# modelscope/dash-infer

Measured on NVIDIA H100. Metric: decode tokens/sec/GPU Qwen2-7B int4-IQ b=1..64; HBM GB/s vs roofline, higher is better.
Workload: dtype bf16 activations x int4 weights (fp32 accumulate), none KV

## Files before the change

### dash-infer_b200/csrc/wq_gemm.cu

```cuda
#include <cstdio>
#include <cstdlib>
#include <cstring>
#include <map>
#include <mutex>
#include <new>

#include "b2_common.cuh"
#include "comm_shared.cuh"
#include "wq_gemm_shared.cuh"

namespace b2 {

constexpr int kWarps = 8;
constexpr int kThreads = kWarps * 32 + 32;
constexpr int kStageBytes = 8192;
static_assert(kBN == kWarps * 16, "one n16 tile per consumer warp");

struct GemmParams {
  const uint8_t* packed;
  const float2* sz;
  const __nv_bfloat16* A;
  int64_t lda;
  __nv_bfloat16* C;
  int64_t ldc;
  const __nv_bfloat16* bias;
  const __nv_bfloat16* residual;
  float* ws;
  unsigned* counters;
  int M, N, K, Np, KT, NG, S;
  int group_tiles;
  int quanta;
  int xt;
  int nst_log2;
  int act;
  float alpha;
  const float* norm_sumsq;
  const __nv_bfloat16* norm_gamma;
  int norm_parts;
  int cluster;
  int norm_self;
  float norm_inv_hidden, norm_eps;
  float* sumsq_out;
  int comm_on;
  CommDev comm;
};

template <int WBITS>
struct WTraits {
  static constexpr int LB = WBITS == 4 ? 16 : (WBITS == 8 ? 32 : 64);
  static constexpr int NCH = LB / 16;
  static constexpr int TILE_BYTES = kWarps * 32 * LB;
  static constexpr int TPS = kStageBytes / TILE_BYTES > 0 ? kStageBytes / TILE_BYTES : 1;
  static constexpr int STAGE_BYTES = TPS * TILE_BYTES;
};

__device__ __forceinline__ void named_bar_sync(int id, int n) { asm volatile("bar.sync %0, %1;" ::"r"(id), "r"(n) : "memory"); }

template <int WBITS, int MT, bool H>
__device__ __forceinline__ void tile_mma(float (&acc)[MT][4], uint32_t wtile, uint32_t woff0, uint32_t woff1, uint32_t xaddr,
                                         int XS8) {
  uint4 xb[MT][2];
#pragma unroll
  for (int m = 0; m < MT; ++m) {
    xb[m][0] = lds128(xaddr + m * XS8);
    xb[m][1] = lds128(xaddr + m * XS8 + 16);
  }
  if (WBITS == 4) {
    const uint2 w0 = lds64(wtile + woff0), w1 = lds64(wtile + woff1);
    const uint32_t r0w[2] = {w0.x, w0.y}, r1w[2] = {w1.x, w1.y};
#pragma unroll
    for (int j = 0; j < 2; ++j) {
      const uint32_t u = r0w[j], v = r1w[j];
      const uint32_t p0 = lop3_and_or(u, kMask4, Ft<H>::kMagic), q0 = lop3_and_or(v, kMask4, Ft<H>::kMagic);
      const uint32_t p1 = lop3_and_or(__funnelshift_r(u, u, 4), kMask4, Ft<H>::kMagic), q1 = lop3_and_or(__funnelshift_r(v, v, 4), kMask4, Ft<H>::kMagic);
      const uint32_t p2 = lop3_and_or(__funnelshift_r(u, u, 8), kMask4, Ft<H>::kMagic), q2 = lop3_and_or(__funnelshift_r(v, v, 8), kMask4, Ft<H>::kMagic);
      const uint32_t p3 = lop3_and_or(__funnelshift_r(u, u, 12), kMask4, Ft<H>::kMagic), q3 = lop3_and_or(__funnelshift_r(v, v, 12), kMask4, Ft<H>::kMagic);
#pragma unroll
      for (int m = 0; m < MT; ++m) {
        Ft<H>::mma(acc[m], p0, q0, p1, q1, xb[m][j].x, xb[m][j].y);
        Ft<H>::mma(acc[m], p2, q2, p3, q3, xb[m][j].z, xb[m][j].w);
      }
    }
  } else if (WBITS == 8) {
    const uint4 w0 = lds128(wtile + woff0), w1 = lds128(wtile + woff1);
    const uint32_t r0w[4] = {w0.x, w0.y, w0.z, w0.w}, r1w[4] = {w1.x, w1.y, w1.z, w1.w};
#pragma unroll
    for (int j = 0; j < 4; ++j) {
      const uint32_t u = r0w[j], v = r1w[j];
      const uint32_t l0 = lop3_and_or(u, kMask4, Ft<H>::kMagic), m0 = lop3_and_or(v, kMask4, Ft<H>::kMagic);
      const uint32_t h0 = lop3_and_or(__funnelshift_r(u, u, 4), kMask4, Ft<H>::kMagicHi), n0 = lop3_and_or(__funnelshift_r(v, v, 4), kMask4, Ft<H>::kMagicHi);
      const uint32_t l1 = lop3_and_or(__funnelshift_r(u, u, 8), kMask4, Ft<H>::kMagic), m1 = lop3_and_or(__funnelshift_r(v, v, 8), kMask4, Ft<H>::kMagic);
      const uint32_t h1 = lop3_and_or(__funnelshift_r(u, u, 12), kMask4, Ft<H>::kMagicHi), n1 = lop3_and_or(__funnelshift_r(v, v, 12), kMask4, Ft<H>::kMagicHi);
#pragma unroll
      for (int m = 0; m < MT; ++m) {
        const uint32_t b0 = (j & 1) ? xb[m][j >> 1].z : xb[m][j >> 1].x;
        const uint32_t b1 = (j & 1) ? xb[m][j >> 1].w : xb[m][j >> 1].y;
        Ft<H>::mma(acc[m], l0, m0, l1, m1, b0, b1);
        Ft<H>::mma(acc[m], h0, n0, h1, n1, b0, b1);
      }
    }
  } else {
#pragma unroll
    for (int u = 0; u < 2; ++u) {
      const uint4 w0 = lds128(wtile + woff0 + u * 2048), w1 = lds128(wtile + woff1 + u * 2048);
#pragma unroll
      for (int m = 0; m < MT; ++m) {
        Ft<H>::mma(acc[m], w0.x, w1.x, w0.y, w1.y, xb[m][u].x, xb[m][u].y);
        Ft<H>::mma(acc[m], w0.z, w1.z, w0.w, w1.w, xb[m][u].z, xb[m][u].w);
      }
    }
  }
}

B2_TRACE_DECL(g_gemv_tr)
#ifdef B2_TRACE
extern "C" int b2_debug_trace_gemv(unsigned long long* host_out) { return (int)cudaMemcpyFromSymbol(host_out, g_gemv_tr, sizeof(g_gemv_tr)); }
#endif

template <int WBITS, int MT, bool GROUPED, bool H>
__global__ void __launch_bounds__(kThreads) wq_gemm_kernel(const GemmParams p) {
  using T = WTraits<WBITS>;
  using F = Ft<H>;
  constexpr int MP = 8 * MT;
  const int NST = 1 << p.nst_log2;
  extern __shared__ __align__(128) uint8_t smem[];
  const int tid = threadIdx.x;
  const int warp = tid >> 5, lane = tid & 31;
  const int g = lane >> 2, t = lane & 3;

  const int ng = blockIdx.x / p.S;
  const int s = blockIdx.x - ng * p.S;
  const int gt = GROUPED ? p.group_tiles : 1;
  const int q0 = (int)((int64_t)s * p.quanta / p.S), q1 = (int)((int64_t)(s + 1) * p.quanta / p.S);
  const int kt0 = q0 * gt, kt1 = q1 * gt;
  const int nt = kt1 - kt0;

  uint8_t* ring = smem;
  const int ring_bytes = NST * T::STAGE_BYTES;
  const int XS = p.xt * 128 + 16;
  uint8_t* xs = ring + ring_bytes;
  uint8_t* grow = xs + MP * XS;
  float* fs = reinterpret_cast<float*>(grow + XS);
  float* suma = fs + MP * kBN;
  const int gpc = GROUPED ? p.xt / gt : 1;
  float* sinv = suma + MP * gpc;
  float* srs = sinv + MP;
  uint64_t* full = reinterpret_cast<uint64_t*>((reinterpret_cast<uintptr_t>(srs + MP + 4) + 7) & ~uintptr_t(7));
  uint64_t* empty = full + NST;
  uint64_t* xbar = empty + NST;
  uint64_t* gbar = xbar + 1;
  __shared__ int s_is_last;

  const bool tr0 = blockIdx.x == 0 && tid == 0;
  if (tr0) B2_TR(g_gemv_tr, 0);
  if (tid == 0) {
    for (int i = 0; i < NST; ++i) {
      mbar_init(&full[i], 1);
      mbar_init(&empty[i], kWarps);
    }
    mbar_init(xbar, 1);
    mbar_init(gbar, 1);
    fence_mbar_init();
  }
  __syncthreads();
  pdl_launch_dependents();
  if (tr0) B2_TR(g_gemv_tr, 1);

  if (warp == kWarps) {
    if (lane == 0) {
      const uint8_t* wsrc = p.packed + ((size_t)ng * p.KT + kt0) * T::TILE_BYTES;
      const int nstages_total = (nt + T::TPS - 1) / T::TPS;
      for (int i = 0; i < nstages_total; ++i) {
        const int slot = i & (NST - 1);
        if (i >= NST) mbar_wait(&empty[slot], ((i >> p.nst_log2) & 1) ^ 1);
        const int tiles = min(T::TPS, nt - i * T::TPS);
        const uint32_t bytes = tiles * T::TILE_BYTES;
        mbar_arrive_expect_tx(&full[slot], bytes);
        bulk_g2s(ring + slot * T::STAGE_BYTES, wsrc + (size_t)i * T::STAGE_BYTES, bytes, &full[slot]);
        if (blockIdx.x == 0 && i == 0) B2_TR(g_gemv_tr, 2);
      }
    }
    return;
  }

  const int n0 = ng * kBN + warp * 16 + g;
  float2 sz0 = make_float2(1.f, 0.f), sz1 = make_float2(1.f, 0.f);
  if (!GROUPED && WBITS != 16) {
    sz0 = p.sz[n0];
    sz1 = p.sz[n0 + 8];
  }

  float acc[MT][4], facc[MT][4];
#pragma unroll
  for (int m = 0; m < MT; ++m)
#pragma unroll
    for (int c = 0; c < 4; ++c) acc[m][c] = facc[m][c] = 0.f;

  for (int i = p.M * XS + tid * 16; i < MP * XS; i += kWarps * 32 * 16) *reinterpret_cast<uint4*>(xs + i) = make_uint4(0, 0, 0, 0);
  const int64_t k_first = (int64_t)kt0 * kBK;
  if (p.norm_self && tid == 0) {
    const int64_t left = ((int64_t)p.K - k_first) * 2;
    const uint32_t gb = (uint32_t)max((int64_t)0, min((int64_t)min(p.xt, nt) * 128, left));
    mbar_arrive_expect_tx(gbar, gb);
    if (gb) bulk_g2s(grow, p.norm_gamma + k_first, gb, gbar);
  }

  pdl_wait();
  if (tr0) B2_TR(g_gemv_tr, 3);

  if (p.norm_sumsq) {
    for (int m = warp; m < MP; m += kWarps) {
      float ss = 0.f;
      if (m < p.M)
        for (int i = lane; i < p.norm_parts; i += 32) ss += __ldcg(p.norm_sumsq + (size_t)i * p.M + m);
#pragma unroll
      for (int o = 16; o > 0; o >>= 1) ss += __shfl_xor_sync(0xffffffffu, ss, o);
      if (lane == 0) sinv[m] = rsqrtf(ss * p.norm_inv_hidden + p.norm_eps);
    }
    named_bar_sync(1, kWarps * 32);
  }
  const uint32_t w_ring = smem_u32(ring);
  const int wc = WBITS == 4 ? (t >> 1) : (WBITS == 8 ? t : 2 * t);
  const int wr = warp * 16 + g;
  const uint32_t woff0 = wc * 2048 + ((wr ^ tile_swz(WBITS, wc)) << 4) + (WBITS == 4 ? 8 * (t & 1) : 0);
  const uint32_t woff1 = wc * 2048 + (((wr + 8) ^ tile_swz(WBITS, wc)) << 4) + (WBITS == 4 ? 8 * (t & 1) : 0);
  const uint32_t x_thr = smem_u32(xs) + g * XS + t * 32;
  const int XS8 = 8 * XS;
  int stage_i = 0;

  for (int xc0 = 0; xc0 < nt; xc0 += p.xt) {
    const int xn = min(p.xt, nt - xc0);
    if (xc0 > 0) named_bar_sync(1, kWarps * 32);
    if (!(p.norm_self || p.M <= 2)) {
      const int64_t kbase = (int64_t)(kt0 + xc0) * kBK;
      const int nvec = xn * 8;
      const int gvec = GROUPED ? gt * 8 : nvec;
      for (int m = warp; m < MP; m += kWarps) {
        const __nv_bfloat16* arow = p.A + (int64_t)m * p.lda + kbase;
        uint8_t* xrow = xs + m * XS;
        const bool mrow = m < p.M;
        for (int v0 = 0, gi = 0; v0 < nvec; v0 += gvec, ++gi) {
          float sacc = 0.f;
          for (int v = v0 + lane; v < v0 + gvec; v += 32) {
            uint4 val = make_uint4(0, 0, 0, 0);
            if (mrow && kbase + v * 8 < p.K) {
              val = *reinterpret_cast<const uint4*>(arow + v * 8);
              if (p.norm_sumsq) {
                const uint4 gv = *reinterpret_cast<const uint4*>(p.norm_gamma + kbase + v * 8);
                const float inv = sinv[m];
                val.x = F::pack(F::lo(val.x) * inv * F::lo(gv.x), F::hi(val.x) * inv * F::hi(gv.x));
                val.y = F::pack(F::lo(val.y) * inv * F::lo(gv.y), F::hi(val.y) * inv * F::hi(gv.y));
                val.z = F::pack(F::lo(val.z) * inv * F::lo(gv.z), F::hi(val.z) * inv * F::hi(gv.z));
                val.w = F::pack(F::lo(val.w) * inv * F::lo(gv.w), F::hi(val.w) * inv * F::hi(gv.w));
              }
            }
            *reinterpret_cast<uint4*>(xrow + v * 16) = val;
            sacc += (F::lo(val.x) + F::hi(val.x)) + (F::lo(val.y) + F::hi(val.y)) +
                    (F::lo(val.z) + F::hi(val.z)) + (F::lo(val.w) + F::hi(val.w));
          }
#pragma unroll
          for (int o = 16; o > 0; o >>= 1) sacc += __shfl_xor_sync(0xffffffffu, sacc, o);
          if (lane == 0) {
            if (GROUPED) suma[m * gpc + gi] = sacc;
            else suma[m] = (xc0 == 0 ? 0.f : suma[m]) + sacc;
          }
        }
      }
    } else
    {
      const int64_t kbase = (int64_t)(kt0 + xc0) * kBK;
      const int chunk = xc0 / p.xt;
      const uint32_t rb = (uint32_t)max((int64_t)0, min((int64_t)xn * 128, ((int64_t)p.K - kbase) * 2));
      if (warp == 0) {
        if (lane == 0) {
          fence_proxy_async();
          if (p.norm_self && xc0 > 0) {
            mbar_arrive_expect_tx(gbar, rb);
            if (rb) bulk_g2s(grow, p.norm_gamma + kbase, rb, gbar);
          }
          mbar_arrive_expect_tx(xbar, rb * p.M);
        }
        __syncwarp();
        if (rb && lane < p.M) bulk_g2s(xs + lane * XS, p.A + (int64_t)lane * p.lda + kbase, rb, xbar);
      }
      if (tr0 && xc0 == 0) B2_TR(g_gemv_tr, 12);
      mbar_wait(xbar, chunk & 1);
      if (p.norm_self) mbar_wait(gbar, chunk & 1);
      if (tr0 && xc0 == 0) B2_TR(g_gemv_tr, 13);
      const int nvec = xn * 8;
      const int gvec = GROUPED ? gt * 8 : nvec;
      const int lvec = rb >> 4;
      for (int m = warp; m < MP; m += kWarps) {
        uint8_t* xrow = xs + m * XS;
        const bool mrow = m < p.M;
        float ssq = 0.f;
        for (int v0 = 0, gi = 0; v0 < nvec; v0 += gvec, ++gi) {
          float sacc = 0.f;
          if (mrow) {
            for (int v = v0 + lane; v < v0 + gvec; v += 32) {
              uint4 val = make_uint4(0, 0, 0, 0);
              if (v < lvec) {
                val = *reinterpret_cast<const uint4*>(xrow + v * 16);
                if (p.norm_self) {
                  const uint4 gv = *reinterpret_cast<const uint4*>(grow + v * 16);
                  const float x0 = F::lo(val.x), x1 = F::hi(val.x), x2 = F::lo(val.y), x3 = F::hi(val.y);
                  const float x4 = F::lo(val.z), x5 = F::hi(val.z), x6 = F::lo(val.w), x7 = F::hi(val.w);
                  ssq += (x0 * x0 + x1 * x1) + (x2 * x2 + x3 * x3) + (x4 * x4 + x5 * x5) + (x6 * x6 + x7 * x7);
                  val.x = F::pack(x0 * F::lo(gv.x), x1 * F::hi(gv.x));
                  val.y = F::pack(x2 * F::lo(gv.y), x3 * F::hi(gv.y));
                  val.z = F::pack(x4 * F::lo(gv.z), x5 * F::hi(gv.z));
                  val.w = F::pack(x6 * F::lo(gv.w), x7 * F::hi(gv.w));
                  *reinterpret_cast<uint4*>(xrow + v * 16) = val;
                } else if (p.norm_sumsq) {
                  const uint4 gv = *reinterpret_cast<const uint4*>(p.norm_gamma + kbase + v * 8);
                  const float inv = sinv[m];
                  val.x = F::pack(F::lo(val.x) * inv * F::lo(gv.x), F::hi(val.x) * inv * F::hi(gv.x));
                  val.y = F::pack(F::lo(val.y) * inv * F::lo(gv.y), F::hi(val.y) * inv * F::hi(gv.y));
                  val.z = F::pack(F::lo(val.z) * inv * F::lo(gv.z), F::hi(val.z) * inv * F::hi(gv.z));
                  val.w = F::pack(F::lo(val.w) * inv * F::lo(gv.w), F::hi(val.w) * inv * F::hi(gv.w));
                  *reinterpret_cast<uint4*>(xrow + v * 16) = val;
                }
              } else {
                *reinterpret_cast<uint4*>(xrow + v * 16) = val;
              }
              sacc += (F::lo(val.x) + F::hi(val.x)) + (F::lo(val.y) + F::hi(val.y)) +
                      (F::lo(val.z) + F::hi(val.z)) + (F::lo(val.w) + F::hi(val.w));
            }
#pragma unroll
            for (int o = 16; o > 0; o >>= 1) sacc += __shfl_xor_sync(0xffffffffu, sacc, o);
          }
          if (lane == 0) {
            if (GROUPED) suma[m * gpc + gi] = sacc;
            else suma[m] = (xc0 == 0 ? 0.f : suma[m]) + sacc;
          }
        }
        if (p.norm_self) {
#pragma unroll
          for (int o = 16; o > 0; o >>= 1) ssq += __shfl_xor_sync(0xffffffffu, ssq, o);
          if (lane == 0) sinv[m] = (xc0 == 0 ? 0.f : sinv[m]) + ssq;
        }
      }
    }
    if (tr0 && xc0 == 0) B2_TR(g_gemv_tr, 14);
    named_bar_sync(1, kWarps * 32);
    if (tr0 && xc0 == 0) B2_TR(g_gemv_tr, 4);

    int gcount = 0;
    for (int xs0 = 0; xs0 < xn; xs0 += T::TPS, ++stage_i) {
      const int slot = stage_i & (NST - 1);
      mbar_wait(&full[slot], (stage_i >> p.nst_log2) & 1);
      if (tr0 && stage_i == 0) B2_TR(g_gemv_tr, 5);
      const uint32_t wst = w_ring + slot * T::STAGE_BYTES;
#pragma unroll
      for (int ti = 0; ti < T::TPS; ++ti) {
        if (T::TPS > 1 && xs0 + ti >= xn) break;
        if (GROUPED && gcount == 0) {
          const int grp = (kt0 + xc0 + xs0 + ti) / gt;
          sz0 = p.sz[(size_t)grp * p.Np + n0];
          sz1 = p.sz[(size_t)grp * p.Np + n0 + 8];
        }
        tile_mma<WBITS, MT, H>(acc, wst + ti * T::TILE_BYTES, woff0, woff1, x_thr + (xs0 + ti) * 128, XS8);
        if (GROUPED && ++gcount == gt) {
          gcount = 0;
          const int gi = (xs0 + ti) / gt;
#pragma unroll
          for (int m = 0; m < MT; ++m) {
#pragma unroll
            for (int c = 0; c < 4; ++c) {
              const float2 z = (c < 2) ? sz0 : sz1;
              const float sa = suma[(m * 8 + 2 * t + (c & 1)) * gpc + gi];
              facc[m][c] += z.x * (acc[m][c] - z.y * sa);
              acc[m][c] = 0.f;
            }
          }
        }
      }
      __syncwarp();
      if (lane == 0) mbar_arrive(&empty[slot]);
    }
  }

  if (tr0) B2_TR(g_gemv_tr, 6);
#pragma unroll
  for (int m = 0; m < MT; ++m) {
#pragma unroll
    for (int c = 0; c < 4; ++c) {
      float v;
      if (WBITS == 16) v = acc[m][c];
      else if (GROUPED) v = facc[m][c];
      else {
        const float2 z = (c < 2) ? sz0 : sz1;
        const float sa = suma[m * 8 + 2 * t + (c & 1)];
        v = z.x * (acc[m][c] - z.y * sa);
      }
      fs[(m * 8 + 2 * t + (c & 1)) * kBN + warp * 16 + g + (c >> 1) * 8] = v;
    }
  }
  named_bar_sync(1, kWarps * 32);

  const int ctid = tid;
  const int MPK = MP * kBN;
  if (p.cluster) {
    if (tr0) B2_TR(g_gemv_tr, 7);
    cluster_arrive();
    cluster_wait();
    if (tr0) B2_TR(g_gemv_tr, 8);
    const uint32_t fs_a = smem_u32(fs), sinv_a = smem_u32(sinv);
    if (p.norm_self) {
      if (ctid < MP) {
        float ss = 0.f;
        for (int r = 0; r < p.S; ++r) ss += ld_dsmem_f(dsmem_addr(sinv_a + ctid * 4, r));
        srs[ctid] = rsqrtf(ss * p.norm_inv_hidden + p.norm_eps);
      }
      named_bar_sync(1, kWarps * 32);
    }
    auto slice_sum = [&](int elem) {
      float4 a = make_float4(0.f, 0.f, 0.f, 0.f);
      for (int r0 = 0; r0 < p.S; r0 += 4) {
        float4 b[4];
#pragma unroll
        for (int r = 0; r < 4; ++r)
          b[r] = r0 + r < p.S ? ld_dsmem_f4(dsmem_addr(fs_a + elem * 4, r0 + r)) : make_float4(0.f, 0.f, 0.f, 0.f);
#pragma unroll
        for (int r = 0; r < 4; ++r) { a.x += b[r].x; a.y += b[r].y; a.z += b[r].z; a.w += b[r].w; }
      }
      return a;
    };
    const bool gather = p.comm_on || p.sumsq_out != nullptr;
    if (!gather) {
      if (p.act == B2_ACT_SWIGLU) {
        for (int i = s + p.S * ctid; i < p.M * 16; i += p.S * kWarps * 32) {
          const int m = i >> 4, cg = i & 15;
          const int n = ng * 64 + cg * 4;
          if (n >= p.N) continue;
          const float4 gq = slice_sum(m * kBN + cg * 4), uq = slice_sum(m * kBN + 64 + cg * 4);
          const float ra = p.norm_self ? p.alpha * srs[m] : p.alpha;
          const float v[4] = {apply_act<B2_ACT_SILU>(gq.x * ra) * (uq.x * ra), apply_act<B2_ACT_SILU>(gq.y * ra) * (uq.y * ra),
                              apply_act<B2_ACT_SILU>(gq.z * ra) * (uq.z * ra), apply_act<B2_ACT_SILU>(gq.w * ra) * (uq.w * ra)};
          __nv_bfloat16* cp = p.C + (int64_t)m * p.ldc + n;
          if (n + 3 < p.N && (reinterpret_cast<uintptr_t>(cp) & 7) == 0) {
            *reinterpret_cast<uint2*>(cp) = make_uint2(F::pack(v[0], v[1]), F::pack(v[2], v[3]));
          } else {
#pragma unroll
            for (int j = 0; j < 4; ++j)
              if (n + j < p.N) cp[j] = F::from_f(v[j]);
          }
        }
      } else {
        for (int i = s + p.S * ctid; i < p.M * 32; i += p.S * kWarps * 32) {
          const int m = i >> 5, c = (i & 31) * 4;
          const int n = ng * kBN + c;
          if (n >= p.N) continue;
          const float4 q = slice_sum(m * kBN + c);
          const float ra = p.norm_self ? p.alpha * srs[m] : p.alpha;
          float v[4] = {q.x * ra, q.y * ra, q.z * ra, q.w * ra};
          __nv_bfloat16* cp = p.C + (int64_t)m * p.ldc + n;
          const __nv_bfloat16* rp = p.residual ? p.residual + (int64_t)m * p.ldc + n : nullptr;
#pragma unroll
          for (int j = 0; j < 4; ++j) {
            if (n + j < p.N) {
              if (p.bias) v[j] += F::to_f(p.bias[n + j]);
              v[j] = apply_act_rt(v[j], p.act);
              if (rp) v[j] += F::to_f(rp[j]);
            }
          }
          if (n + 3 < p.N && (reinterpret_cast<uintptr_t>(cp) & 7) == 0) {
            *reinterpret_cast<uint2*>(cp) = make_uint2(F::pack(v[0], v[1]), F::pack(v[2], v[3]));
          } else {
#pragma unroll
            for (int j = 0; j < 4; ++j)
              if (n + j < p.N) cp[j] = F::from_f(v[j]);
          }
        }
      }
      if (tr0) B2_TR(g_gemv_tr, 10);
      cluster_arrive();
      cluster_wait();
      if (tr0) B2_TR(g_gemv_tr, 11);
      return;
    }
    if (s == 0) {
      for (int i = ctid; i < p.M * 32; i += kWarps * 32) {
        const float4 q = slice_sum(i * 4);
        *reinterpret_cast<float4*>(fs + i * 4) = q;
      }
    }
    cluster_arrive();
    cluster_wait();
    if (s != 0) return;
  } else if (p.S > 1) {
    float* wsu = p.ws + ((size_t)ng * p.S + s) * MPK;
    for (int i = ctid * 4; i < p.M * kBN; i += kWarps * 32 * 4)
      *reinterpret_cast<float4*>(wsu + i) = *reinterpret_cast<const float4*>(fs + i);
    float* wsq = p.ws + (size_t)p.NG * p.S * MPK;
    if (p.norm_self && ctid < p.M) wsq[((size_t)ng * p.S + s) * MP + ctid] = sinv[ctid];
    __threadfence();
    named_bar_sync(1, kWarps * 32);
    if (tr0) B2_TR(g_gemv_tr, 7);
    if (ctid == 0) {
      const unsigned prev = atomicAdd(&p.counters[ng], 1u);
      s_is_last = (prev == (unsigned)(p.S - 1));
    }
    named_bar_sync(1, kWarps * 32);
    if (tr0) B2_TR(g_gemv_tr, 8);
    if (!s_is_last) return;
    __threadfence();
    if (ng == 0 && ctid == 0) B2_TR(g_gemv_tr, 9);
    const float* wsg = p.ws + (size_t)ng * p.S * MPK;
    float ssq_l = 0.f;
    float ssq_h = 0.f;
    if (p.norm_self) {
      if (lane < p.S && warp < p.M) ssq_l = __ldcg(wsq + ((size_t)ng * p.S + lane) * MP + warp);
      if (lane < p.S && warp + kWarps < p.M) ssq_h = __ldcg(wsq + ((size_t)ng * p.S + lane) * MP + warp + kWarps);
    }
    for (int i = ctid * 4; i < p.M * kBN; i += kWarps * 32 * 4) {
      float4 a = make_float4(0.f, 0.f, 0.f, 0.f);
      for (int s0 = 0; s0 < p.S; s0 += 8) {
        float4 b[8];
#pragma unroll
        for (int u = 0; u < 8; ++u)
          b[u] = (s0 + u < p.S) ? __ldcg(reinterpret_cast<const float4*>(wsg + (size_t)(s0 + u) * MPK + i))
                                : make_float4(0.f, 0.f, 0.f, 0.f);
#pragma unroll
        for (int u = 0; u < 8; ++u) { a.x += b[u].x; a.y += b[u].y; a.z += b[u].z; a.w += b[u].w; }
      }
      *reinterpret_cast<float4*>(fs + i) = a;
    }
    if (p.norm_self) {
#pragma unroll
      for (int o = 16; o > 0; o >>= 1) {
        ssq_l += __shfl_xor_sync(0xffffffffu, ssq_l, o);
        ssq_h += __shfl_xor_sync(0xffffffffu, ssq_h, o);
      }
      if (lane == 0) {
        sinv[warp] = ssq_l;
        if (MP > kWarps) sinv[warp + kWarps] = ssq_h;
      }
    }
    if (ctid == 0) p.counters[ng] = 0;
    named_bar_sync(1, kWarps * 32);
    if (ng == 0 && ctid == 0) B2_TR(g_gemv_tr, 10);
  }

  if (p.norm_self && !p.cluster) {
    if (ctid < MP) srs[ctid] = rsqrtf(sinv[ctid] * p.norm_inv_hidden + p.norm_eps);
    named_bar_sync(1, kWarps * 32);
  }
  if (p.act == B2_ACT_SWIGLU) {
    for (int i = ctid; i < p.M * 32; i += kWarps * 32) {
      const int m = i >> 5, np = i & 31;
      const int n = ng * 64 + np * 2;
      if (n >= p.N) continue;
      const float ra = p.norm_self ? p.alpha * srs[m] : p.alpha;
      const float g0 = fs[m * kBN + np * 2] * ra, g1 = fs[m * kBN + np * 2 + 1] * ra;
      const float u0 = fs[m * kBN + 64 + np * 2] * ra, u1 = fs[m * kBN + 64 + np * 2 + 1] * ra;
      const float v0 = apply_act<B2_ACT_SILU>(g0) * u0, v1 = apply_act<B2_ACT_SILU>(g1) * u1;
      __nv_bfloat16* cp = p.C + (int64_t)m * p.ldc + n;
      if ((n + 1) < p.N && ((reinterpret_cast<uintptr_t>(cp) & 3) == 0)) *reinterpret_cast<uint32_t*>(cp) = F::pack(v0, v1);
      else {
        cp[0] = F::from_f(v0);
        if ((n + 1) < p.N) cp[1] = F::from_f(v1);
      }
    }
    return;
  }
  if (p.comm_on) {
    const CommDev& cd = p.comm;
    const unsigned epoch = *reinterpret_cast<volatile unsigned*>(cd.epoch);
    const unsigned want = epoch + 1;
    const int par = epoch & 1;
    const size_t my_slot = comm_slot_offset(cd, par, cd.rank);
    for (int i = ctid; i < p.M * (kBN / 2); i += kWarps * 32) {
      const int m = i >> 6, np = i & 63;
      const int n = ng * kBN + np * 2;
      if (n >= p.N) continue;
      float v0 = fs[m * kBN + np * 2] * p.alpha, v1 = fs[m * kBN + np * 2 + 1] * p.alpha;
      if (p.bias) {
        v0 += F::to_f(p.bias[n]);
        v1 += F::to_f(p.bias[n + 1]);
      }
      const uint32_t pk = F::pack(v0, v1);
      const size_t off = my_slot + ((size_t)m * p.N + n) * 2;
      for (int r = 0; r < cd.nranks; ++r) *reinterpret_cast<uint32_t*>(cd.peer[(cd.rank + r) % cd.nranks] + off) = pk;
    }
    __threadfence_system();
    named_bar_sync(1, kWarps * 32);
    __shared__ int s_comm_ok;
    if (ctid == 0) s_comm_ok = 1;
    if (ctid < cd.nranks) {
      unsigned* f = reinterpret_cast<unsigned*>(cd.peer[ctid] + comm_flag_offset(cd, par, cd.rank, ng));
      asm volatile("st.release.sys.global.u32 [%0], %1;" ::"l"(f), "r"(want) : "memory");
    }
    named_bar_sync(1, kWarps * 32);
    if (ctid < cd.nranks) {
      const unsigned* f = reinterpret_cast<const unsigned*>(cd.peer[cd.rank] + comm_flag_offset(cd, par, ctid, ng));
      if (!wait_flag(f, want, cd.timeout_ns, cd.error)) s_comm_ok = 0;
    }
    named_bar_sync(1, kWarps * 32);
    if (s_comm_ok) {
      const uint8_t* base = cd.peer[cd.rank];
      for (int i = ctid; i < p.M * (kBN / 2); i += kWarps * 32) {
        const int m = i >> 6, np = i & 63;
        const int n = ng * kBN + np * 2;
        if (n >= p.N) continue;
        const size_t eo = ((size_t)m * p.N + n) * 2;
        float a0 = 0.f, a1 = 0.f;
        for (int r = 0; r < cd.nranks; ++r) {
          const uint32_t v = __ldcg(reinterpret_cast<const uint32_t*>(base + comm_slot_offset(cd, par, r) + eo));
          a0 += F::lo(v);
          a1 += F::hi(v);
        }
        if (p.residual) {
          const uint32_t v = *reinterpret_cast<const uint32_t*>(p.residual + (int64_t)m * p.ldc + n);
          a0 += F::lo(v);
          a1 += F::hi(v);
        }
        *reinterpret_cast<uint32_t*>(p.C + (int64_t)m * p.ldc + n) = F::pack(a0, a1);
      }
    }
    named_bar_sync(1, kWarps * 32);
    if (ctid == 0) {
      __threadfence();
      if (atomicAdd(cd.done, 1u) == (unsigned)(p.NG - 1)) {
        *cd.done = 0;
        __threadfence();
        *reinterpret_cast<volatile unsigned*>(cd.epoch) = want;
      }
    }
    return;
  }
  for (int i = ctid; i < p.M * (kBN / 2); i += kWarps * 32) {
    const int m = i >> 6, np = i & 63;
    const int n = ng * kBN + np * 2;
    if (n >= p.N) continue;
    const float ra = p.norm_self ? p.alpha * srs[m] : p.alpha;
    float v0 = fs[m * kBN + np * 2] * ra, v1 = fs[m * kBN + np * 2 + 1] * ra;
    const bool has1 = (n + 1) < p.N;
    if (p.bias) {
      v0 += F::to_f(p.bias[n]);
      if (has1) v1 += F::to_f(p.bias[n + 1]);
    }
    v0 = apply_act_rt(v0, p.act);
    v1 = apply_act_rt(v1, p.act);
    __nv_bfloat16* cp = p.C + (int64_t)m * p.ldc + n;
    if (p.residual) {
      const __nv_bfloat16* rp = p.residual + (int64_t)m * p.ldc + n;
      v0 += F::to_f(rp[0]);
      if (has1) v1 += F::to_f(rp[1]);
    }
    if (has1 && ((reinterpret_cast<uintptr_t>(cp) & 3) == 0)) {
      *reinterpret_cast<uint32_t*>(cp) = F::pack(v0, v1);
    } else {
      cp[0] = F::from_f(v0);
      if (has1) cp[1] = F::from_f(v1);
    }
    if (p.sumsq_out) {
      fs[m * kBN + np * 2] = F::to_f(F::from_f(v0));
      fs[m * kBN + np * 2 + 1] = has1 ? F::to_f(F::from_f(v1)) : 0.f;
    }
  }
  if (ng == 0 && ctid == 0) B2_TR(g_gemv_tr, 11);
  if (p.sumsq_out) {
    named_bar_sync(1, kWarps * 32);
    for (int m = warp; m < p.M; m += kWarps) {
      float ss = 0.f;
#pragma unroll
      for (int i = 0; i < kBN / 32; ++i) {
        const int c = lane + 32 * i;
        const float v = (ng * kBN + c) < p.N ? fs[m * kBN + c] : 0.f;
        ss += v * v;
      }
#pragma unroll
      for (int o = 16; o > 0; o >>= 1) ss += __shfl_xor_sync(0xffffffffu, ss, o);
      if (lane == 0) p.sumsq_out[(size_t)ng * p.M + m] = ss;
    }
  }
}

__global__ void pack_w4_kernel(uint32_t* __restrict__ dst, const uint8_t* __restrict__ q, const uint8_t* __restrict__ q2, int pair,
                               int K, int N, int KT, int NG) {
  const int64_t total = (int64_t)NG * KT * 1024;
  const int npack = (N + 1) / 2;
  for (int64_t i = blockIdx.x * (int64_t)blockDim.x + threadIdx.x; i < total; i += (int64_t)gridDim.x * blockDim.x) {
    const int j = i & 3;
    const int rs = (i >> 2) & 127;
    const int c = (i >> 9) & 1;
    const int64_t tile = i >> 10;
    const int kt = tile % KT, ng = tile / KT;
    const int r = rs ^ tile_swz(4, c);
    const int n = pair ? ng * 64 + (r & 63) : ng * kBN + r;
    const uint8_t* qs = (pair && r >= 64) ? q2 : q;
    uint32_t word = 0;
    for (int nb = 0; nb < 8; ++nb) {
      const int k = kt * kBK + 32 * c + 8 * j + 2 * (nb & 3) + (nb >> 2);
      uint32_t v = 0;
      if (n < N && k < K) {
        const uint8_t b = qs[(int64_t)k * npack + (n >> 1)];
        v = (n & 1) ? (b >> 4) : (b & 0xF);
      }
      word |= v << (4 * nb);
    }
    dst[i] = (word << 3) | (word >> 29);
  }
}

__global__ void pack_w8_kernel(uint32_t* __restrict__ dst, const uint8_t* __restrict__ q, const uint8_t* __restrict__ q2, int pair,
                               int K, int N, int KT, int NG, int is_signed) {
  const int64_t total = (int64_t)NG * KT * 2048;
  for (int64_t i = blockIdx.x * (int64_t)blockDim.x + threadIdx.x; i < total; i += (int64_t)gridDim.x * blockDim.x) {
    const int j = i & 3;
    const int rs = (i >> 2) & 127;
    const int c = (i >> 9) & 3;
    const int64_t tile = i >> 11;
    const int kt = tile % KT, ng = tile / KT;
    const int r = rs ^ tile_swz(8, c);
    const int n = pair ? ng * 64 + (r & 63) : ng * kBN + r;
    const uint8_t* qs = (pair && r >= 64) ? q2 : q;
    uint32_t word = 0;
    for (int b = 0; b < 4; ++b) {
      const int kk = (b == 0) ? 0 : (b == 2 ? 1 : (b == 1 ? 2 : 3));
      const int k = kt * kBK + 16 * c + 4 * j + kk;
      uint32_t v = is_signed ? 0x80u : 0u;
      if (n < N && k < K) v = qs[(int64_t)k * N + n] ^ (is_signed ? 0x80u : 0u);
      word |= v << (8 * b);
    }
    dst[i] = (word << 3) | (word >> 29);
  }
}

__global__ void pack_w16_kernel(uint32_t* __restrict__ dst, const uint16_t* __restrict__ wsrc, const uint16_t* __restrict__ wsrc2,
                                int pair, int K, int N, int KT, int NG) {
  const int64_t total = (int64_t)NG * KT * 4096;
  for (int64_t i = blockIdx.x * (int64_t)blockDim.x + threadIdx.x; i < total; i += (int64_t)gridDim.x * blockDim.x) {
    const int j = i & 3;
    const int rs = (i >> 2) & 127;
    const int c = (i >> 9) & 7;
    const int64_t tile = i >> 12;
    const int kt = tile % KT, ng = tile / KT;
    const int r = rs ^ tile_swz(16, c);
    const int n = pair ? ng * 64 + (r & 63) : ng * kBN + r;
    const uint16_t* ws = (pair && r >= 64) ? wsrc2 : wsrc;
    uint32_t word = 0;
    for (int e = 0; e < 2; ++e) {
      const int k = kt * kBK + 8 * c + 2 * j + e;
      uint32_t v = 0;
      if (n < N && k < K) v = ws[(int64_t)k * N + n];
      word |= v << (16 * e);
    }
    dst[i] = word;
  }
}

__global__ void pack_sz_kernel(float2* __restrict__ dst, const __nv_bfloat16* __restrict__ scales,
                               const __nv_bfloat16* __restrict__ zeros, const __nv_bfloat16* __restrict__ scales2,
                               const __nv_bfloat16* __restrict__ zeros2, int pair, int G, int N, int Np, float zbias, int fp16) {
  const int64_t total = (int64_t)G * Np;
  for (int64_t i = blockIdx.x * (int64_t)blockDim.x + threadIdx.x; i < total; i += (int64_t)gridDim.x * blockDim.x) {
    const int np = i % Np, gi = i / Np;
    const int r = np & (kBN - 1), ng = np / kBN;
    const int n = pair ? ng * 64 + (r & 63) : np;
    const __nv_bfloat16* sc = (pair && r >= 64) ? scales2 : scales;
    const __nv_bfloat16* zr = (pair && r >= 64) ? zeros2 : zeros;
    float2 v = make_float2(0.f, 0.f);
    if (n < N) {
      const __nv_bfloat16 sv = sc[(int64_t)gi * N + n], zv = zr[(int64_t)gi * N + n];
      v = fp16 ? make_float2(Ft<true>::to_f(sv), Ft<true>::to_f(zv) + zbias) : make_float2(Ft<false>::to_f(sv), Ft<false>::to_f(zv) + zbias);
    }
    dst[i] = v;
  }
}

}

using namespace b2;

struct Plan {
  bool valid = false;
  int S = 1, xt = 1, smem = 0, quanta = 1, nst_log2 = 2;
  bool cluster = false;
};

struct b2_gemm_wq {
  b2_gemm_wq_desc d;
  int Kp = 0, Np = 0, KT = 0, NG = 0, G = 1, group_tiles = 0;
  int group_k = 0;
  size_t tile_bytes = 0, packed_bytes = 0;
  void* packed = nullptr;
  bool own_packed = false;
  float2* sz = nullptr;
  bool own_sz = false;
  unsigned* counters = nullptr;
  Plan plans[2];
  int tc_S = 0;
  int tc_S2 = 0;
  bool pair = false;
  int device = 0;
};

typedef void (*gemm_kernel_t)(const GemmParams);

template <int WBITS, bool GROUPED, bool H>
static gemm_kernel_t pick_mt(int mt) {
  switch (mt) {
    case 1: return wq_gemm_kernel<WBITS, 1, GROUPED, H>;
    default: return wq_gemm_kernel<WBITS, 2, GROUPED, H>;
  }
}
template <bool H>
static gemm_kernel_t pick_kernel_ft(int wbits, bool grouped, int mt) {
  if (wbits == 4) return grouped ? pick_mt<4, true, H>(mt) : pick_mt<4, false, H>(mt);
  if (wbits == 8) return grouped ? pick_mt<8, true, H>(mt) : pick_mt<8, false, H>(mt);
  return pick_mt<16, false, H>(mt);
}
static gemm_kernel_t pick_kernel(int wbits, bool grouped, int mt, bool fp16) {
  return fp16 ? pick_kernel_ft<true>(wbits, grouped, mt) : pick_kernel_ft<false>(wbits, grouped, mt);
}
static int stage_bytes_of(int wbits) { return wbits == 16 ? WTraits<16>::STAGE_BYTES : kStageBytes; }
static int tile_bytes_of(int wbits) { return wbits == 4 ? WTraits<4>::TILE_BYTES : (wbits == 8 ? WTraits<8>::TILE_BYTES : WTraits<16>::TILE_BYTES); }

static int env_int(const char* name, int dflt) {
  const char* v = getenv(name);
  return v ? atoi(v) : dflt;
}

cudaError_t b2::raise_smem_limit(const void* kern, int smem) {
  static std::mutex mu;
  static std::map<const void*, int> limit;
  std::lock_guard<std::mutex> lk(mu);
  int& cur = limit[kern];
  if (smem <= cur) return cudaSuccess;
  cudaError_t e = cudaFuncSetAttribute(kern, cudaFuncAttributeMaxDynamicSharedMemorySize, smem);
  if (e == cudaSuccess) cur = smem;
  return e;
}

static int make_plan(b2_gemm_wq* h, int mti) {
  Plan& pl = h->plans[mti];
  if (pl.valid) return B2_OK;
  const int mt = 1 << mti, MP = 8 * mt;
  const bool grouped = h->group_tiles > 0;
  const int gt = grouped ? h->group_tiles : 1;
  const int quanta = h->KT / gt;
  const int sms = sm_count();
  gemm_kernel_t kern = pick_kernel(h->d.wbits, grouped, mt, h->d.ft == B2_DT_F16);
  const int ring_kb = env_int("B2_GEMM_RING_KB", 32);
  auto log2_stages = [&](int kb) {
    int l = 1;
    while ((2 << l) * stage_bytes_of(h->d.wbits) <= kb * 1024) ++l;
    return l;
  };
  int nst_log2 = log2_stages(ring_kb);
  const int tps = kStageBytes / tile_bytes_of(h->d.wbits) > 0 ? kStageBytes / tile_bytes_of(h->d.wbits) : 1;
  const int xq = gt > tps ? gt : tps;
  const int x_budget = env_int("B2_GEMM_XBYTES", 20 * 1024);
  int xt_cap = (x_budget / (MP + 1) - 16) / 128;
  xt_cap = xt_cap / xq * xq;
  if (xt_cap < xq) xt_cap = xq;
  auto smem_for = [&](int xt, int nl2) {
    const int gpc = grouped ? xt / gt : 1;
    return (1 << nl2) * stage_bytes_of(h->d.wbits) + (MP + 1) * (xt * 128 + 16) + MP * kBN * 4 + MP * gpc * 4 + 2 * MP * 4 + 16 + 8 +
           (1 << nl2) * 16 + 16 + 64;
  };
  int smem = smem_for(xt_cap, nst_log2);
  B2_CUDA_TRY(raise_smem_limit((const void*)kern, smem));
  int occ = 1;
  B2_CUDA_TRY(cudaOccupancyMaxActiveBlocksPerMultiprocessor(&occ, kern, kThreads, smem));
  if (occ < 1) occ = 1;
  const int want = env_int("B2_GEMM_CTAS_PER_SM", 4);
  if (want > 0 && occ > want) occ = want;
  const int slots = occ * sms;
  int S = slots / h->NG;
  const int min_quanta = (2 + gt - 1) / gt;
  if (S > quanta / (min_quanta > 0 ? min_quanta : 1)) S = quanta / (min_quanta > 0 ? min_quanta : 1);
  const int smax = env_int("B2_GEMM_MAX_SPLIT", 32);
  if (S > smax) S = smax;
  if (S < 1) S = 1;
  const int force = env_int("B2_GEMM_FORCE_SPLIT", 0);
  if (force > 0) S = force < quanta ? force : quanta;
  if (S > 32) S = 32;
  bool cluster = false;
  if (env_int("B2_GEMM_CLUSTER", 1) && force <= 0 && S > 1) {
    int sc = 2;
    while (sc * 2 <= S && sc * 2 <= 8) sc *= 2;
    while (sc > 1 && !cluster) {
      if (h->NG * sc * 4 < sms * 3) break;
      const int nl2 = h->NG * sc <= 2 * sms ? log2_stages(env_int("B2_GEMM_CLUSTER_RING_KB", 64)) : nst_log2;
      const int sm_c = smem_for(xt_cap, nl2);
      B2_CUDA_TRY(raise_smem_limit((const void*)kern, sm_c));
      cudaLaunchConfig_t cfg{};
      cfg.gridDim = dim3(h->NG * sc);
      cfg.blockDim = dim3(kThreads);
      cfg.dynamicSmemBytes = sm_c;
      cudaLaunchAttribute at[1];
      at[0].id = cudaLaunchAttributeClusterDimension;
      at[0].val.clusterDim.x = sc;
      at[0].val.clusterDim.y = 1;
      at[0].val.clusterDim.z = 1;
      cfg.attrs = at;
      cfg.numAttrs = 1;
      int ncl = 0;
      if (cudaOccupancyMaxActiveClusters(&ncl, kern, &cfg) == cudaSuccess && ncl >= h->NG) {
        cluster = true;
        S = sc;
        nst_log2 = nl2;
      } else {
        (void)cudaGetLastError();
        sc >>= 1;
      }
    }
  }
  const int unit_tiles = ((quanta + S - 1) / S) * gt;
  int xt = unit_tiles < xt_cap ? unit_tiles : xt_cap;
  xt = (xt + xq - 1) / xq * xq;
  pl.S = S;
  pl.xt = xt;
  pl.nst_log2 = nst_log2;
  pl.cluster = cluster;
  pl.smem = smem_for(xt, nst_log2);
  pl.quanta = quanta;
  pl.valid = true;
  return B2_OK;
}

extern "C" {

int b2_gemm_wq_create(b2_gemm_wq_t* out, const b2_gemm_wq_desc* d) {
  if (!out || !d) return B2_ERR_PARAM;
  if (d->K <= 0 || d->N <= 0 || d->max_m <= 0) return B2_ERR_PARAM;
  if (d->wbits != 4 && d->wbits != 8 && d->wbits != 16) return B2_ERR_PARAM;
  if (d->ft != B2_DT_BF16 && d->ft != B2_DT_F16) return B2_ERR_UNSUPPORTED;
  if (d->wbits == 4 && d->qtype != B2_DT_U8) return B2_ERR_PARAM;
  if (d->wbits == 8 && d->qtype != B2_DT_U8 && d->qtype != B2_DT_I8) return B2_ERR_PARAM;
  if (d->K % 8 != 0) return B2_ERR_UNSUPPORTED;
  bool general_groups = false;
  if (d->wbits != 16 && d->group_size != -1) {
    if (d->group_size <= 0) return B2_ERR_UNSUPPORTED;
    if (d->group_size % kBK != 0) {
      if (d->wbits != 4 || d->group_size % 8 != 0 || d->group_size < 32 || d->reserved == 1) return B2_ERR_UNSUPPORTED;
      general_groups = true;
    }
  }
  b2_gemm_wq* h = new (std::nothrow) b2_gemm_wq();
  if (!h) return B2_ERR_RUNTIME;
  h->d = *d;
  const bool grouped = d->wbits != 16 && d->group_size != -1;
  const int kq = (grouped && !general_groups) ? d->group_size : kBK;
  h->Kp = (d->K + kq - 1) / kq * kq;
  h->pair = d->reserved == 1;
  h->Np = h->pair ? (d->N + 63) / 64 * kBN : (d->N + kBN - 1) / kBN * kBN;
  h->KT = h->Kp / kBK;
  h->NG = h->Np / kBN;
  h->group_tiles = (grouped && !general_groups) ? d->group_size / kBK : 0;
  h->group_k = general_groups ? d->group_size : 0;
  h->G = grouped ? (general_groups ? (d->K + d->group_size - 1) / d->group_size : h->Kp / d->group_size) : 1;
  h->tile_bytes = tile_bytes_of(d->wbits);
  h->packed_bytes = (size_t)h->NG * h->KT * h->tile_bytes;
  cudaGetDevice(&h->device);
  cudaError_t e = cudaMalloc(&h->counters, sizeof(unsigned) * h->NG);
  if (e == cudaSuccess) e = cudaMemset(h->counters, 0, sizeof(unsigned) * h->NG);
  if (e != cudaSuccess) {
    set_last_error("b2_gemm_wq_create", e);
    delete h;
    return B2_ERR_CUDA;
  }
  *out = h;
  return B2_OK;
}

int b2_gemm_wq_destroy(b2_gemm_wq_t h) {
  if (!h) return B2_OK;
  if (h->own_packed && h->packed) cudaFree(h->packed);
  if (h->own_sz && h->sz) cudaFree(h->sz);
  if (h->counters) cudaFree(h->counters);
  delete h;
  return B2_OK;
}

size_t b2_gemm_wq_packed_bytes(b2_gemm_wq_t h) { return h ? h->packed_bytes : 0; }

static int prepare_impl(b2_gemm_wq_t h, const void* qdata, const void* scales, const void* zeros, const void* qdata2,
                        const void* scales2, const void* zeros2, void* packed_dst, void* stream_) {
  if (!h || !qdata) return B2_ERR_PARAM;
  cudaStream_t stream = (cudaStream_t)stream_;
  const b2_gemm_wq_desc& d = h->d;
  const int pair = h->pair ? 1 : 0;
  if (pair && !qdata2) return B2_ERR_PARAM;
  if (d.wbits != 16 && (!scales || !zeros || (pair && (!scales2 || !zeros2)))) return B2_ERR_PARAM;
  if (packed_dst) {
    if (h->own_packed && h->packed) cudaFree(h->packed);
    h->packed = packed_dst;
    h->own_packed = false;
  } else if (!h->packed || !h->own_packed) {
    B2_CUDA_TRY(cudaMalloc(&h->packed, h->packed_bytes));
    h->own_packed = true;
  }
  const int threads = 256;
  const int64_t words = (int64_t)h->packed_bytes / 4;
  const int blocks = (int)((words + threads - 1) / threads > 65535 * 8 ? 65535 * 8 : (words + threads - 1) / threads);
  if (d.wbits == 4)
    pack_w4_kernel<<<blocks, threads, 0, stream>>>((uint32_t*)h->packed, (const uint8_t*)qdata, (const uint8_t*)qdata2, pair, d.K, d.N,
                                                   h->KT, h->NG);
  else if (d.wbits == 8)
    pack_w8_kernel<<<blocks, threads, 0, stream>>>((uint32_t*)h->packed, (const uint8_t*)qdata, (const uint8_t*)qdata2, pair, d.K, d.N,
                                                   h->KT, h->NG, d.qtype == B2_DT_I8);
  else
    pack_w16_kernel<<<blocks, threads, 0, stream>>>((uint32_t*)h->packed, (const uint16_t*)qdata, (const uint16_t*)qdata2, pair, d.K,
                                                    d.N, h->KT, h->NG);
  if (int st = launch_failed("pack_weights")) return st;
  if (d.wbits != 16) {
    if (!h->sz || !h->own_sz) {
      B2_CUDA_TRY(cudaMalloc(&h->sz, sizeof(float2) * (size_t)h->G * h->Np));
      h->own_sz = true;
    }
    const float b0 = d.ft == B2_DT_F16 ? 128.f : 16.f;
    const float zbias = d.wbits == 4 ? b0 : (d.qtype == B2_DT_I8 ? 17.f * b0 + 128.f : 17.f * b0);
    const int64_t tot = (int64_t)h->G * h->Np;
    pack_sz_kernel<<<(int)((tot + 255) / 256), 256, 0, stream>>>(h->sz, (const __nv_bfloat16*)scales, (const __nv_bfloat16*)zeros,
                                                                 (const __nv_bfloat16*)scales2, (const __nv_bfloat16*)zeros2, pair,
                                                                 h->G, d.N, h->Np, zbias, d.ft == B2_DT_F16 ? 1 : 0);
    if (int st = launch_failed("pack_sz")) return st;
  }
  return B2_OK;
}

int b2_gemm_wq_prepare_weights(b2_gemm_wq_t h, const void* qdata, const void* scales, const void* zeros,
                               void* packed_dst, void* stream_) {
  if (h && h->pair) return B2_ERR_PARAM;
  return prepare_impl(h, qdata, scales, zeros, nullptr, nullptr, nullptr, packed_dst, stream_);
}

int b2_gemm_wq_prepare_swiglu(b2_gemm_wq_t h, const void* q_gate, const void* s_gate, const void* z_gate, const void* q_up,
                              const void* s_up, const void* z_up, void* stream_) {
  if (!h || !h->pair) return B2_ERR_PARAM;
  return prepare_impl(h, q_gate, s_gate, z_gate, q_up, s_up, z_up, nullptr, stream_);
}

int b2_gemm_wq_attach_packed(b2_gemm_wq_t h, const void* packed, const void* scales_f32, const void* zeros_f32) {
  (void)zeros_f32;
  if (!h || !packed) return B2_ERR_PARAM;
  if (h->own_packed && h->packed) cudaFree(h->packed);
  h->packed = const_cast<void*>(packed);
  h->own_packed = false;
  if (scales_f32) {
    if (h->own_sz && h->sz) cudaFree(h->sz);
    h->sz = (float2*)const_cast<void*>(scales_f32);
    h->own_sz = false;
  }
  return B2_OK;
}

static int mt_index_for(int M) { return M <= 8 ? 0 : 1; }

constexpr int kTcMinM = 17;

static bool use_tc(const b2_gemm_wq* h, int M) {
  if (h->group_k > 0) return true;
  return M >= kTcMinM && (h->group_tiles == 0 || h->d.wbits == 4);
}

static int make_tc_plan(b2_gemm_wq* h) {
  if (h->tc_S > 0) return B2_OK;
  const int ctas = env_int("B2_GEMM_TC_CTAS_PER_SM", 1);
  auto split_for = [&](int slots, int smax) {
    int S = slots / h->NG;
    if (S > h->KT / 4) S = h->KT / 4;
    if (S > smax) S = smax;
    return S < 1 ? 1 : S;
  };
  h->tc_S = split_for(ctas * sm_count(), env_int("B2_GEMM_TC_MAX_SPLIT", 6));
  h->tc_S2 = split_for(env_int("B2_GEMM_TC_DUAL_SLOTS", 2) * sm_count(), env_int("B2_GEMM_TC_MAX_SPLIT2", 8));
  return B2_OK;
}

static bool tc_dual(const b2_gemm_wq* h) {
  static const int on = env_int("B2_GEMM_TC_DUAL", 1);
  if (!on || h->d.wbits != 4) return false;
  return on >= 2 || h->NG >= 2 * sm_count();
}

size_t b2_gemm_wq_workspace_bytes(b2_gemm_wq_t h, int M) {
  if (!h || M <= 0) return 0;
  if (use_tc(h, M)) {
    if (make_tc_plan(h) != B2_OK) return 0;
    const int sm = h->tc_S > h->tc_S2 ? h->tc_S : h->tc_S2;
    return sm <= 1 ? 16 : (size_t)h->NG * sm * kTcMaxM * kBN * sizeof(float) + 16;
  }
  const int mc = M > kGemvMaxM ? kGemvMaxM : M;
  const int mti = mt_index_for(mc);
  if (make_plan(h, mti) != B2_OK) return 0;
  const Plan& pl = h->plans[mti];
  if (pl.S <= 1 || pl.cluster) return 16;
  return (size_t)h->NG * pl.S * (8 << mti) * (kBN + 1) * sizeof(float) + 16;
}

size_t b2_gemm_wq_algo_bytes(b2_gemm_wq_t h, int M) {
  if (!h) return 0;
  const b2_gemm_wq_desc& d = h->d;
  const size_t mul = h->pair ? 2 : 1;
  size_t w = mul * (size_t)d.K * d.N * d.wbits / 8;
  size_t prm = d.wbits == 16 ? 0 : mul * (size_t)2 * 2 * h->G * d.N;
  return w + prm + (size_t)2 * M * ((size_t)d.K + d.N);
}

int b2_gemm_wq_sumsq_parts(b2_gemm_wq_t h) { return h ? h->NG : 0; }

int b2_gemm_wq_run(b2_gemm_wq_t h, const void* A, int64_t lda, void* C, int64_t ldc, int M, const void* bias,
                   const void* residual, int activation, float alpha, void* workspace, size_t workspace_bytes,
                   void* stream_) {
  return b2_gemm_wq_run_fused(h, A, lda, C, ldc, M, bias, residual, activation, alpha, workspace, workspace_bytes, nullptr, stream_);
}

extern "C" const void* b2_comm_device_view(b2_comm_t c);

static int run_impl(b2_gemm_wq_t h, const void* A, int64_t lda, void* C, int64_t ldc, int M, const void* bias,
                    const void* residual, int activation, float alpha, void* workspace, size_t workspace_bytes,
                    const b2_gemm_fuse* fuse, const CommDev* comm, void* stream_);

int b2_gemm_wq_run_fused(b2_gemm_wq_t h, const void* A, int64_t lda, void* C, int64_t ldc, int M, const void* bias,
                         const void* residual, int activation, float alpha, void* workspace, size_t workspace_bytes,
                         const b2_gemm_fuse* fuse, void* stream_) {
  return run_impl(h, A, lda, C, ldc, M, bias, residual, activation, alpha, workspace, workspace_bytes, fuse, nullptr, stream_);
}

int b2_gemm_wq_run_fp8(b2_gemm_wq_t h, const void* A8, int64_t lda_bytes, const float* a_scale, const float* tile_sums, void* C,
                       int64_t ldc, int M, const void* bias, const void* residual, int activation, float alpha, void* workspace,
                       size_t workspace_bytes, void* stream_) {
  if (!h || !A8 || !a_scale || !tile_sums || !C || M <= 0) return B2_ERR_PARAM;
  if (!h->packed) return B2_ERR_RUNTIME;
  if (M > h->d.max_m) return B2_ERR_LIMIT;
  if (h->d.wbits != 4 || h->group_tiles > 0 || h->group_k > 0 || h->d.ft != B2_DT_BF16) return B2_ERR_UNSUPPORTED;
  if (h->pair != (activation == B2_ACT_SWIGLU)) return B2_ERR_PARAM;
  if (activation != B2_ACT_SWIGLU && (activation < 0 || activation > B2_ACT_SIGMOID)) return B2_ERR_PARAM;
  if (h->pair && (bias || residual)) return B2_ERR_UNSUPPORTED;
  if ((reinterpret_cast<uintptr_t>(A8) & 15) || (lda_bytes % 16) != 0 || lda_bytes < h->d.K) return B2_ERR_UNSUPPORTED;
  if (int st = make_tc_plan(h)) return st;
  const size_t need = h->tc_S <= 1 ? 16 : (size_t)h->NG * h->tc_S * kTcMaxM * kBN * sizeof(float) + 16;
  if (workspace_bytes < need || (h->tc_S > 1 && !workspace)) return B2_ERR_PARAM;
  for (int m0 = 0; m0 < M; m0 += kTcMaxM) {
    TcLaunch a;
    a.packed = (const uint8_t*)h->packed; a.sz = h->sz;
    a.A = reinterpret_cast<const __nv_bfloat16*>((const uint8_t*)A8 + (int64_t)m0 * lda_bytes); a.lda = lda_bytes;
    a.C = (__nv_bfloat16*)C + (int64_t)m0 * ldc; a.ldc = ldc;
    a.bias = (const __nv_bfloat16*)bias;
    a.residual = residual ? (const __nv_bfloat16*)residual + (int64_t)m0 * ldc : nullptr;
    a.ws = (float*)workspace; a.counters = h->counters;
    a.M = (M - m0) > kTcMaxM ? kTcMaxM : (M - m0);
    a.N = h->d.N; a.K = h->d.K; a.Np = h->Np; a.KT = h->KT; a.NG = h->NG; a.S = h->tc_S;
    a.act = activation; a.alpha = alpha;
    a.a_scale = a_scale + m0; a.tile_sums = tile_sums + (size_t)m0 * h->KT;
    cudaError_t e = tc_launch(4, a, (cudaStream_t)stream_);
    if (e != cudaSuccess) {
      set_last_error("wq_gemm_tc (fp8) launch", e);
      return B2_ERR_CUDA;
    }
  }
  return B2_OK;
}

int b2_gemm_wq_run_allreduce(b2_gemm_wq_t h, const void* A, int64_t lda, void* C, int64_t ldc, int M, const void* bias,
                             const void* residual, float alpha, void* workspace, size_t workspace_bytes, b2_comm_t comm,
                             void* stream_) {
  const CommDev* cd = static_cast<const CommDev*>(b2_comm_device_view(comm));
  if (!h || !cd) return B2_ERR_PARAM;
  for (int r = 0; r < cd->nranks; ++r)
    if (!cd->peer[r]) return B2_ERR_RUNTIME;
  if (M > 16 || h->pair || (h->d.N & 1) || ldc != h->d.N || h->NG > kCommMaxChunks) return B2_ERR_UNSUPPORTED;
  if ((size_t)M * h->d.N * 2 > cd->max_bytes) return B2_ERR_LIMIT;
  if (((uintptr_t)C & 3) || (residual && ((uintptr_t)residual & 3))) return B2_ERR_UNSUPPORTED;
  return run_impl(h, A, lda, C, ldc, M, bias, residual, B2_ACT_NONE, alpha, workspace, workspace_bytes, nullptr, cd, stream_);
}

static int run_impl(b2_gemm_wq_t h, const void* A, int64_t lda, void* C, int64_t ldc, int M, const void* bias,
                    const void* residual, int activation, float alpha, void* workspace, size_t workspace_bytes,
                    const b2_gemm_fuse* fuse, const CommDev* comm, void* stream_) {
  if (!h || !A || !C || M <= 0) return B2_ERR_PARAM;
  const bool norm_self = fuse && !fuse->norm_sumsq && fuse->norm_gamma;
  const bool fused = fuse && (fuse->norm_sumsq || fuse->sumsq_out || norm_self || fuse->xg_out);
  if (fused && use_tc(h, M) && !comm) {
    const bool cons = fuse->norm_sumsq != nullptr, prod = fuse->xg_out != nullptr;
    if (norm_self || (cons && fuse->norm_gamma) || (fuse->sumsq_out && !prod)) return B2_ERR_UNSUPPORTED;
    if (cons && (fuse->norm_parts <= 0 || fuse->norm_hidden <= 0)) return B2_ERR_PARAM;
    if (prod) {
      if (!fuse->sumsq_out || !fuse->gamma_out || h->pair || activation != B2_ACT_NONE) return B2_ERR_PARAM;
      if ((h->d.N & 3) || (ldc & 3) || (fuse->ldxg & 3) || (reinterpret_cast<uintptr_t>(C) & 7) ||
          (reinterpret_cast<uintptr_t>(fuse->xg_out) & 7) || (reinterpret_cast<uintptr_t>(fuse->gamma_out) & 7) ||
          (residual && (reinterpret_cast<uintptr_t>(residual) & 7)) || (bias && (reinterpret_cast<uintptr_t>(bias) & 7)))
        return B2_ERR_UNSUPPORTED;
    }
  } else {
    if (norm_self && (fuse->norm_hidden != h->d.K || comm)) return B2_ERR_PARAM;
    if (norm_self && (reinterpret_cast<uintptr_t>(fuse->norm_gamma) & 15)) return B2_ERR_UNSUPPORTED;
    if (fused && (M > 16 || (h->pair && fuse->sumsq_out) || fuse->xg_out)) return B2_ERR_UNSUPPORTED;
    if (fuse && fuse->norm_sumsq && (!fuse->norm_gamma || fuse->norm_parts <= 0 || fuse->norm_hidden <= 0)) return B2_ERR_PARAM;
  }
  if (!h->packed) return B2_ERR_RUNTIME;
  if (M > h->d.max_m) return B2_ERR_LIMIT;
  if (h->group_k > 0 && comm) return B2_ERR_UNSUPPORTED;
  if (h->pair != (activation == B2_ACT_SWIGLU)) return B2_ERR_PARAM;
  if (activation != B2_ACT_SWIGLU && (activation < 0 || activation > B2_ACT_SIGMOID)) return B2_ERR_PARAM;
  if (h->pair && (bias || residual)) return B2_ERR_UNSUPPORTED;
  if ((reinterpret_cast<uintptr_t>(A) & 15) || (lda % 8) != 0) return B2_ERR_UNSUPPORTED;
  if (workspace_bytes < b2_gemm_wq_workspace_bytes(h, M)) return B2_ERR_PARAM;
  cudaStream_t stream = (cudaStream_t)stream_;
  const bool grouped = h->group_tiles > 0;
  if (use_tc(h, M) && !comm) {
    if (int st = make_tc_plan(h)) return st;
    const bool dual = tc_dual(h);
    const int tcs = dual ? h->tc_S2 : h->tc_S;
    if (tcs > 1 && !workspace) return B2_ERR_PARAM;
    for (int m0 = 0; m0 < M; m0 += kTcMaxM) {
      TcLaunch a;
      a.dual = dual;
      a.fp16 = h->d.ft == B2_DT_F16;
      a.packed = (const uint8_t*)h->packed; a.sz = h->sz;
      a.A = (const __nv_bfloat16*)A + (int64_t)m0 * lda; a.lda = lda;
      a.C = (__nv_bfloat16*)C + (int64_t)m0 * ldc; a.ldc = ldc;
      a.bias = (const __nv_bfloat16*)bias;
      a.residual = residual ? (const __nv_bfloat16*)residual + (int64_t)m0 * ldc : nullptr;
      a.ws = (float*)workspace; a.counters = h->counters;
      a.M = (M - m0) > kTcMaxM ? kTcMaxM : (M - m0);
      a.N = h->d.N; a.K = h->d.K; a.Np = h->Np; a.KT = h->KT; a.NG = h->NG; a.S = tcs;
      a.act = activation; a.alpha = alpha;
      a.group_tiles = h->group_tiles;
      a.group_k = h->group_k; a.ngroups = h->G;
      if (fused) {
        a.norm_ld = M;
        if (fuse->norm_sumsq) {
          a.norm_sumsq = fuse->norm_sumsq + m0; a.norm_parts = fuse->norm_parts;
          a.norm_inv_hidden = 1.0f / (float)fuse->norm_hidden; a.norm_eps = fuse->norm_eps;
        }
        if (fuse->xg_out) {
          a.sumsq_out = fuse->sumsq_out + m0;
          a.xg_out = (__nv_bfloat16*)fuse->xg_out + (int64_t)m0 * fuse->ldxg;
          a.gamma_out = (const __nv_bfloat16*)fuse->gamma_out; a.ldxg = fuse->ldxg;
        }
      }
      cudaError_t e = tc_launch(h->d.wbits, a, stream);
      if (e != cudaSuccess) {
        set_last_error("wq_gemm_tc launch", e);
        return B2_ERR_CUDA;
      }
    }
    return B2_OK;
  }
  if (h->d.wbits == 16 && M <= kGemvMaxM && !fused && !comm && h->d.ft == B2_DT_BF16) {
    Gemv2Launch a;
    a.packed = (const uint8_t*)h->packed;
    a.A = (const __nv_bfloat16*)A; a.lda = lda;
    a.C = (__nv_bfloat16*)C; a.ldc = ldc;
    a.bias = (const __nv_bfloat16*)bias;
    a.residual = (const __nv_bfloat16*)residual;
    a.M = M; a.N = h->d.N; a.K = h->d.K; a.KT = h->KT; a.NG = h->NG;
    a.pair = h->pair; a.act = activation; a.alpha = alpha;
    Gemv2Plan pl;
    if (gemv2_plan(a, &pl)) {
      cudaError_t e = gemv2_launch(a, pl, stream);
      if (e != cudaSuccess) {
        set_last_error("wq_gemv2 launch", e);
        return B2_ERR_CUDA;
      }
      return B2_OK;
    }
  }
  for (int m0 = 0; m0 < M; m0 += kGemvMaxM) {
    const int mc = (M - m0) > kGemvMaxM ? kGemvMaxM : (M - m0);
    const int mti = mt_index_for(mc);
    if (int st = make_plan(h, mti)) return st;
    const Plan& pl = h->plans[mti];
    if (pl.S > 1 && !pl.cluster && !workspace) return B2_ERR_PARAM;
    GemmParams p;
    p.packed = (const uint8_t*)h->packed;
    p.sz = h->sz;
    p.A = (const __nv_bfloat16*)A + (int64_t)m0 * lda;
    p.lda = lda;
    p.C = (__nv_bfloat16*)C + (int64_t)m0 * ldc;
    p.ldc = ldc;
    p.bias = (const __nv_bfloat16*)bias;
    p.residual = residual ? (const __nv_bfloat16*)residual + (int64_t)m0 * ldc : nullptr;
    p.ws = (float*)workspace;
    p.counters = h->counters;
    p.M = mc; p.N = h->d.N; p.K = h->d.K; p.Np = h->Np; p.KT = h->KT; p.NG = h->NG; p.S = pl.S;
    p.group_tiles = h->group_tiles;
    p.quanta = pl.quanta;
    p.xt = pl.xt;
    p.nst_log2 = pl.nst_log2;
    p.act = activation;
    p.alpha = alpha;
    p.norm_sumsq = fuse ? fuse->norm_sumsq : nullptr;
    p.norm_gamma = fuse ? (const __nv_bfloat16*)fuse->norm_gamma : nullptr;
    p.norm_parts = fuse ? fuse->norm_parts : 0;
    p.norm_self = norm_self ? 1 : 0;
    p.cluster = pl.cluster ? 1 : 0;
    p.norm_inv_hidden = fuse && fuse->norm_hidden > 0 ? 1.0f / (float)fuse->norm_hidden : 0.f;
    p.norm_eps = fuse ? fuse->norm_eps : 0.f;
    p.sumsq_out = fuse ? fuse->sumsq_out : nullptr;
    p.comm_on = comm ? 1 : 0;
    if (comm) p.comm = *comm;
    else memset(&p.comm, 0, sizeof(p.comm));
    gemm_kernel_t kern = pick_kernel(h->d.wbits, grouped, 1 << mti, h->d.ft == B2_DT_F16);
    cudaError_t e = pl.cluster ? launch_cluster(kern, dim3(h->NG * pl.S), dim3(kThreads), (size_t)pl.smem, stream, true, (unsigned)pl.S, p)
                               : launch(kern, dim3(h->NG * pl.S), dim3(kThreads), (size_t)pl.smem, stream, true, p);
    if (e != cudaSuccess) {
      set_last_error("wq_gemm launch", e);
      return B2_ERR_CUDA;
    }
  }
  return B2_OK;
}

}
```

### dash-infer_b200/csrc/wq_gemm_shared.cuh

```cuda
#pragma once
#include <cuda.h>

#include "b2_common.cuh"

namespace b2 {

constexpr int kBN = 128;
constexpr int kBK = 64;
constexpr uint32_t kMask4 = 0x00780078u;
constexpr uint32_t kMagic = 0x41804180u;
constexpr uint32_t kMagicHi = 0x43804380u;

__host__ __device__ __forceinline__ int tile_swz(int wbits, int c) {
  return wbits == 4 ? 4 * (c & 1) : (wbits == 8 ? 2 * (c & 3) : 2 * ((c >> 1) & 3));
}

struct TcLaunch {
  const uint8_t* packed;
  const float2* sz;
  const __nv_bfloat16* A;
  int64_t lda;
  __nv_bfloat16* C;
  int64_t ldc;
  const __nv_bfloat16* bias;
  const __nv_bfloat16* residual;
  float* ws;
  unsigned* counters;
  int M, N, K, Np, KT, NG, S;
  int act;
  float alpha;
  const float* a_scale = nullptr;
  const float* tile_sums = nullptr;
  int group_tiles = 0;
  int group_k = 0, ngroups = 1;
  bool fp16 = false;
  bool dual = false;
  const float* norm_sumsq = nullptr;
  int norm_parts = 0, norm_ld = 0;
  float norm_inv_hidden = 0.f, norm_eps = 0.f;
  float* sumsq_out = nullptr;
  __nv_bfloat16* xg_out = nullptr;
  const __nv_bfloat16* gamma_out = nullptr;
  int64_t ldxg = 0;
};
struct Gemv2Launch {
  const uint8_t* packed;
  const __nv_bfloat16* A;
  int64_t lda;
  __nv_bfloat16* C;
  int64_t ldc;
  const __nv_bfloat16* bias;
  const __nv_bfloat16* residual;
  int M, N, K, KT, NG;
  bool pair;
  int act;
  float alpha;
};
struct Gemv2Plan {
  int cb_log2, xt, nst_log2, mt, grid, smem;
};
bool gemv2_plan(const Gemv2Launch& a, Gemv2Plan* plan);
cudaError_t gemv2_launch(const Gemv2Launch& a, const Gemv2Plan& plan, cudaStream_t stream);

constexpr int kGemvMaxM = 16;
constexpr int kTcMaxM = 64;
int tc_smem_bytes(int wbits, bool dual);
cudaError_t tc_launch(int wbits, const TcLaunch& a, cudaStream_t stream);

cudaError_t raise_smem_limit(const void* kern, int smem);

typedef CUresult (*EncodeTiledFn)(CUtensorMap*, CUtensorMapDataType, cuuint32_t, void*, const cuuint64_t*, const cuuint64_t*,
                                  const cuuint32_t*, const cuuint32_t*, CUtensorMapInterleave, CUtensorMapSwizzle,
                                  CUtensorMapL2promotion, CUtensorMapFloatOOBfill);
EncodeTiledFn encode_tiled();

}
```

### dash-infer_b200/csrc/wq_gemm_tc.cu

```cuda
#include <cstdlib>

#include "b2_common.cuh"
#include "wq_gemm_shared.cuh"

namespace b2 {

constexpr int kTcThreads = 384;
constexpr int kTcNM = 64;
constexpr int kTcNSW = 6;
constexpr int kTcNSX = 3;
constexpr int kTcXTile = kTcNM * 128;

__device__ __forceinline__ void wg_fence() { asm volatile("wgmma.fence.sync.aligned;" ::: "memory"); }
__device__ __forceinline__ void wg_commit() { asm volatile("wgmma.commit_group.sync.aligned;" ::: "memory"); }
template <int N>
__device__ __forceinline__ void wg_wait() { asm volatile("wgmma.wait_group.sync.aligned %0;" ::"n"(N) : "memory"); }
__device__ __forceinline__ void wg_fence_acc(float (&d)[32]) {
#pragma unroll
  for (int i = 0; i < 32; ++i) asm volatile("" : "+f"(d[i])::"memory");
}
__device__ __forceinline__ uint64_t wg_desc(uint32_t saddr) {
  return (uint64_t)((saddr >> 4) & 0x3FFF) | ((uint64_t)1 << 16) | ((uint64_t)(1024 >> 4) << 32) | ((uint64_t)1 << 62);
}

#define B2_WG_D16 "{%0,%1,%2,%3,%4,%5,%6,%7,%8,%9,%10,%11,%12,%13,%14,%15}"
#define B2_WG_D32                                                                                                          \
  "{%0,%1,%2,%3,%4,%5,%6,%7,%8,%9,%10,%11,%12,%13,%14,%15,%16,%17,%18,%19,%20,%21,%22,%23,%24,%25,%26,%27,%28,%29,%30,%31}"
#define B2_WG_ACC16(d)                                                                                                       \
  "+f"(d[0]), "+f"(d[1]), "+f"(d[2]), "+f"(d[3]), "+f"(d[4]), "+f"(d[5]), "+f"(d[6]), "+f"(d[7]), "+f"(d[8]), "+f"(d[9]), \
      "+f"(d[10]), "+f"(d[11]), "+f"(d[12]), "+f"(d[13]), "+f"(d[14]), "+f"(d[15])
#define B2_WG_ACC32(d)                                                                                                       \
  B2_WG_ACC16(d), "+f"(d[16]), "+f"(d[17]), "+f"(d[18]), "+f"(d[19]), "+f"(d[20]), "+f"(d[21]), "+f"(d[22]), "+f"(d[23]), \
      "+f"(d[24]), "+f"(d[25]), "+f"(d[26]), "+f"(d[27]), "+f"(d[28]), "+f"(d[29]), "+f"(d[30]), "+f"(d[31])

template <int KIND>
__device__ __forceinline__ void wg_mma(float (&d)[32], const uint32_t (&a)[4], uint64_t desc, bool n32) {
  if (n32) {
    if (KIND == 0)
      asm volatile("{\n\t.reg .pred p;\n\tsetp.ne.b32 p, %21, 0;\n\t"
                   "wgmma.mma_async.sync.aligned.m64n32k16.f32.bf16.bf16 " B2_WG_D16 ", {%16,%17,%18,%19}, %20, p, 1, 1, 0;\n\t}"
                   : B2_WG_ACC16(d) : "r"(a[0]), "r"(a[1]), "r"(a[2]), "r"(a[3]), "l"(desc), "r"(1));
    else if (KIND == 1)
      asm volatile("{\n\t.reg .pred p;\n\tsetp.ne.b32 p, %21, 0;\n\t"
                   "wgmma.mma_async.sync.aligned.m64n32k16.f32.f16.f16 " B2_WG_D16 ", {%16,%17,%18,%19}, %20, p, 1, 1, 0;\n\t}"
                   : B2_WG_ACC16(d) : "r"(a[0]), "r"(a[1]), "r"(a[2]), "r"(a[3]), "l"(desc), "r"(1));
    else
      asm volatile("{\n\t.reg .pred p;\n\tsetp.ne.b32 p, %21, 0;\n\t"
                   "wgmma.mma_async.sync.aligned.m64n32k32.f32.e4m3.e4m3 " B2_WG_D16 ", {%16,%17,%18,%19}, %20, p, 1, 1;\n\t}"
                   : B2_WG_ACC16(d) : "r"(a[0]), "r"(a[1]), "r"(a[2]), "r"(a[3]), "l"(desc), "r"(1));
  } else {
    if (KIND == 0)
      asm volatile("{\n\t.reg .pred p;\n\tsetp.ne.b32 p, %37, 0;\n\t"
                   "wgmma.mma_async.sync.aligned.m64n64k16.f32.bf16.bf16 " B2_WG_D32 ", {%32,%33,%34,%35}, %36, p, 1, 1, 0;\n\t}"
                   : B2_WG_ACC32(d) : "r"(a[0]), "r"(a[1]), "r"(a[2]), "r"(a[3]), "l"(desc), "r"(1));
    else if (KIND == 1)
      asm volatile("{\n\t.reg .pred p;\n\tsetp.ne.b32 p, %37, 0;\n\t"
                   "wgmma.mma_async.sync.aligned.m64n64k16.f32.f16.f16 " B2_WG_D32 ", {%32,%33,%34,%35}, %36, p, 1, 1, 0;\n\t}"
                   : B2_WG_ACC32(d) : "r"(a[0]), "r"(a[1]), "r"(a[2]), "r"(a[3]), "l"(desc), "r"(1));
    else
      asm volatile("{\n\t.reg .pred p;\n\tsetp.ne.b32 p, %37, 0;\n\t"
                   "wgmma.mma_async.sync.aligned.m64n64k32.f32.e4m3.e4m3 " B2_WG_D32 ", {%32,%33,%34,%35}, %36, p, 1, 1;\n\t}"
                   : B2_WG_ACC32(d) : "r"(a[0]), "r"(a[1]), "r"(a[2]), "r"(a[3]), "l"(desc), "r"(1));
  }
}

__device__ __forceinline__ uint32_t tc_prmt(uint32_t a, uint32_t b, uint32_t sel) {
  uint32_t d;
  asm("prmt.b32 %0, %1, %2, %3;" : "=r"(d) : "r"(a), "r"(b), "r"(sel));
  return d;
}
__device__ __forceinline__ uint32_t lds32(uint32_t addr) {
  uint32_t v;
  asm volatile("ld.shared.u32 %0, [%1];" : "=r"(v) : "r"(addr));
  return v;
}
__device__ __forceinline__ uint32_t nib4_to_e4m3(uint32_t w_rot3, uint32_t qsh, uint32_t msel) {
  const uint32_t word = __funnelshift_r(w_rot3, w_rot3, 3);
  const uint32_t sel = (word & 0x77777777u) >> qsh;
  const uint32_t T0 = 0x44403800u, T1 = 0x4E4C4A48u, H0 = 0x53525150u, H1 = 0x57565554u;
  const uint32_t lo = tc_prmt(T0, T1, sel), hi = tc_prmt(H0, H1, sel);
  const uint32_t m = tc_prmt(word << 4, word, msel);
  uint32_t r;
  asm("lop3.b32 %0, %1, %2, %3, 0xD8;" : "=r"(r) : "r"(lo), "r"(hi), "r"(m));
  return r;
}

struct TcParams {
  const uint8_t* packed;
  const float2* sz;
  const __nv_bfloat16* A;
  int64_t lda;
  __nv_bfloat16* C;
  int64_t ldc;
  const __nv_bfloat16* bias;
  const __nv_bfloat16* residual;
  float* ws;
  unsigned* counters;
  int M, N, K, Np, KT, NG, S;
  int act;
  float alpha;
  const float* a_scale;
  const float* tile_sums;
  const float* norm_sumsq;
  int norm_parts, norm_ld;
  float norm_inv_hidden, norm_eps;
  float* sumsq_out;
  __nv_bfloat16* xg_out;
  const __nv_bfloat16* gamma_out;
  int64_t ldxg;
  int nm;
  int group_tiles;
  int group_k, ngroups;
};

template <int WBITS, bool MULTI, bool A8 = false, bool GROUPED = false, bool DUAL = false, bool H = false>
__global__ void __launch_bounds__(kTcThreads, DUAL ? 2 : 1) wq_gemm_tc_kernel(const TcParams p, const __grid_constant__ CUtensorMap amap) {
  constexpr int TILE_BYTES = WBITS == 4 ? 4096 : (WBITS == 8 ? 8192 : 16384);
  constexpr int NCH = WBITS == 4 ? 2 : (WBITS == 8 ? 4 : 8);
  constexpr int NSW = WBITS == 16 ? 4 : kTcNSW;
  constexpr int TPS = WBITS == 4 ? (DUAL ? 2 : 4) : 2;
  constexpr int KIND = A8 ? 2 : (H ? 1 : 0);
  static_assert(!A8 || WBITS == 4, "fp8 activations: int4 weights only");
  static_assert(!DUAL || (WBITS == 4 && !A8), "two CTAs per SM: int4 weights, 16-bit activations");
  static_assert(!H || !A8, "fp8 activations come with bf16 outputs");
  using F = Ft<H>;
  static_assert(!GROUPED || (!A8 && WBITS != 16), "sub-channel weights: bf16 activations, int4 / int8");
  const int XTILE_LD = p.nm * 128;
  constexpr int XTPS = A8 ? TPS / 2 : TPS;
  constexpr int WSTAGE = TPS * TILE_BYTES;
  constexpr int XSTAGE = XTPS * kTcXTile;
  extern __shared__ uint8_t smem_raw[];
  uint8_t* smem = reinterpret_cast<uint8_t*>((reinterpret_cast<uintptr_t>(smem_raw) + 1023) & ~uintptr_t(1023));
  uint8_t* xring = smem;
  uint8_t* wring = xring + kTcNSX * XSTAGE;
  float* suma = reinterpret_cast<float*>(wring + NSW * WSTAGE);
  uint64_t* bars = reinterpret_cast<uint64_t*>(suma + kTcNM);
  uint64_t* wfull = bars;
  uint64_t* wfree = wfull + kTcNSW;
  uint64_t* afull = wfree + kTcNSW;
  uint64_t* xsum = afull + kTcNSX;
  uint64_t* xfree = xsum + kTcNSX;
  float* ascale = reinterpret_cast<float*>(bars) + 64;
  __shared__ int s_is_last;

  const int tid = threadIdx.x, warp = tid >> 5, lane = tid & 31;
  const int nunits = p.NG * p.S;

  if (tid == 0) {
    for (int i = 0; i < NSW; ++i) { mbar_init(&wfull[i], 1); mbar_init(&wfree[i], 8); }
    for (int i = 0; i < kTcNSX; ++i) { mbar_init(&afull[i], 1); mbar_init(&xsum[i], 2); mbar_init(&xfree[i], 8); }
    fence_mbar_init();
  }
  __syncthreads();
  pdl_launch_dependents();

  int w_pre = 0;
  const int my_units = !MULTI ? 1 : ((int)blockIdx.x < nunits) ? (nunits - (int)blockIdx.x + (int)gridDim.x - 1) / (int)gridDim.x : 0;
  for (int uit = 0; uit < my_units; ++uit) {
  const int unit = (int)blockIdx.x + uit * (int)gridDim.x;
  const int ng = unit / p.S;
  const int s = unit - ng * p.S;
  const int kt0 = (int)((int64_t)s * p.KT / p.S), kt1 = (int)((int64_t)(s + 1) * p.KT / p.S);
  const int nt = kt1 - kt0;
  const int nst = (nt + TPS - 1) / TPS;
  const int gbase = MULTI ? uit * nst : 0;
  if (warp == 8) {
    if (lane == 0) {
      auto issue = [&](int g, const uint8_t* src, uint32_t bytes) {
        const int slot = g % NSW;
        if (g >= NSW) mbar_wait_backoff(&wfree[slot], ((g / NSW) & 1) ^ 1);
        mbar_arrive_expect_tx(&wfull[slot], bytes);
        bulk_g2s(wring + slot * WSTAGE, src, bytes, &wfull[slot]);
      };
      const uint8_t* wsrc = p.packed + ((size_t)ng * p.KT + kt0) * TILE_BYTES;
      for (int st = w_pre; st < nst; ++st) issue(gbase + st, wsrc + (size_t)st * WSTAGE, min(TPS, nt - st * TPS) * TILE_BYTES);
      w_pre = 0;
      const int nu = unit + gridDim.x;
      if (MULTI && nu < nunits) {
        const int ng2 = nu / p.S, s2 = nu - ng2 * p.S;
        const int k0 = (int)((int64_t)s2 * p.KT / p.S), k1 = (int)((int64_t)(s2 + 1) * p.KT / p.S);
        const int nt2 = k1 - k0, nst2 = (nt2 + TPS - 1) / TPS;
        const uint8_t* wsrc2 = p.packed + ((size_t)ng2 * p.KT + k0) * TILE_BYTES;
        w_pre = min(NSW, nst2);
        for (int st = 0; st < w_pre; ++st)
          issue(gbase + nst + st, wsrc2 + (size_t)st * WSTAGE, min(TPS, nt2 - st * TPS) * TILE_BYTES);
      }
    }
  } else if (warp == 9) {
    if (lane == 0) {
      pdl_wait();
      for (int st = 0; st < nst; ++st) {
        const int g = gbase + st;
        const int slot = g % kTcNSX;
        if (g >= kTcNSX) {
          const uint32_t par = ((g / kTcNSX) & 1) ^ 1;
          mbar_wait_backoff(&xfree[slot], par);
          mbar_wait_backoff(&xsum[slot], par);
        }
        const int wtiles = min(TPS, nt - st * TPS);
        const int tiles = A8 ? (wtiles + 1) / 2 : wtiles;
        mbar_arrive_expect_tx(&afull[slot], tiles * XTILE_LD);
        for (int ti = 0; ti < tiles; ++ti)
          asm volatile("cp.async.bulk.tensor.2d.shared::cluster.global.mbarrier::complete_tx::bytes [%0], [%1, {%2, %3}], [%4];"
                       ::"r"(smem_u32(xring + slot * XSTAGE + ti * kTcXTile)), "l"(reinterpret_cast<uint64_t>(&amap)),
                         "r"((kt0 + st * TPS + (A8 ? 2 * ti : ti)) * kBK), "r"(0), "r"(smem_u32(&afull[slot]))
                       : "memory");
      }
    }
  } else if (warp >= 10) {
    const int xt = tid - 320;
    float r0 = 0.f, r1 = 0.f, r2 = 0.f, r3 = 0.f;
    if (A8) {
      pdl_wait();
      if (xt < p.M) {
        const float* ts = p.tile_sums + (size_t)xt * p.KT;
        for (int kt = kt0; kt < kt1; ++kt) r0 += ts[kt];
        ascale[xt] = p.a_scale[xt];
      } else {
        ascale[xt] = 0.f;
      }
    }
    if (!A8 && p.norm_sumsq) {
      pdl_wait();
      float ss = 0.f;
      if (xt < p.M)
        for (int i = 0; i < p.norm_parts; ++i) ss += __ldcg(p.norm_sumsq + (size_t)i * p.norm_ld + xt);
      ascale[xt] = rsqrtf(ss * p.norm_inv_hidden + p.norm_eps);
    }
    for (int st = 0; st < nst; ++st) {
      const int g = gbase + st;
      const int slot = g % kTcNSX;
      mbar_wait(&afull[slot], (g / kTcNSX) & 1);
      const int tiles = (WBITS == 16 || A8 || GROUPED || xt >= p.nm) ? 0 : min(TPS, nt - st * TPS);
      for (int ti = 0; ti < tiles; ++ti) {
        const uint32_t rbase = smem_u32(xring + slot * XSTAGE + ti * kTcXTile) + xt * 128;
#pragma unroll
        for (int c = 0; c < 8; c += 2) {
          const uint4 v = lds128(rbase + ((c ^ (xt & 7)) << 4));
          const uint4 w = lds128(rbase + (((c + 1) ^ (xt & 7)) << 4));
          r0 += (F::lo(v.x) + F::hi(v.x)) + (F::lo(v.y) + F::hi(v.y));
          r1 += (F::lo(v.z) + F::hi(v.z)) + (F::lo(v.w) + F::hi(v.w));
          r2 += (F::lo(w.x) + F::hi(w.x)) + (F::lo(w.y) + F::hi(w.y));
          r3 += (F::lo(w.z) + F::hi(w.z)) + (F::lo(w.w) + F::hi(w.w));
        }
      }
      __syncwarp();
      if (lane == 0) mbar_arrive(&xsum[slot]);
    }
    suma[xt] = (r0 + r1) + (r2 + r3);
    asm volatile("bar.sync 3, 320;" ::: "memory");
  } else {
    const int wg = warp >> 2, g8 = lane >> 2, t4 = lane & 3;
    const int rr0 = wg * 64 + (warp & 3) * 16 + g8, rr1 = rr0 + 8;
    const bool n32 = p.nm == 32;
    const float2 sz0 = (WBITS == 16 || GROUPED) ? make_float2(1.f, 0.f) : p.sz[ng * kBN + rr0];
    const float2 sz1 = (WBITS == 16 || GROUPED) ? make_float2(1.f, 0.f) : p.sz[ng * kBN + rr1];
    const uint32_t wring_u = smem_u32(wring), xring_u = smem_u32(xring);
    uint32_t off0[NCH], off1[NCH];
#pragma unroll
    for (int c = 0; c < NCH; ++c) {
      off0[c] = c * 2048 + ((rr0 ^ tile_swz(WBITS, c)) << 4);
      off1[c] = c * 2048 + ((rr1 ^ tile_swz(WBITS, c)) << 4);
    }
    const uint32_t sh4 = 4 * t4, sh8 = 8 * (t4 & 1), qsh = 16 * (t4 & 1), msel = (t4 & 1) ? 0xFBEAu : 0xD9C8u;
    const int wa = t4 >> 1;
    auto word = [](const uint4& v, int j) { return j == 0 ? v.x : (j == 1 ? v.y : (j == 2 ? v.z : v.w)); };

    float d[32], dt[32];
#pragma unroll
    for (int i = 0; i < 32; ++i) d[i] = dt[i] = 0.f;
    int prev_xs = -1;
    for (int st = 0; st < nst; ++st) {
      const int g = gbase + st;
      const int slot = g % NSW, xs = g % kTcNSX;
      uint32_t gs2[TPS][2], gc2[TPS][2];
      if (GROUPED && p.group_k == 0) {
#pragma unroll
        for (int ti = 0; ti < TPS; ++ti) {
          const int kt = min(kt0 + st * TPS + ti, kt1 - 1);
          const float2 z0 = __ldg(p.sz + (size_t)(kt / p.group_tiles) * p.Np + ng * kBN + rr0);
          const float2 z1 = __ldg(p.sz + (size_t)(kt / p.group_tiles) * p.Np + ng * kBN + rr1);
          const float c0 = (F::kBias + 8.f - z0.y) * z0.x, c1 = (F::kBias + 8.f - z1.y) * z1.x;
          if (DUAL) {
            gs2[ti][0] = F::pack(z0.x, z1.x);
            gc2[ti][0] = F::pack(c0, c1);
          } else {
            gs2[ti][0] = F::pack(z0.x, z0.x); gs2[ti][1] = F::pack(z1.x, z1.x);
            gc2[ti][0] = F::pack(c0, c0); gc2[ti][1] = F::pack(c1, c1);
          }
        }
      }
      mbar_wait(&wfull[slot], (g / NSW) & 1);
      mbar_wait(&afull[xs], (g / kTcNSX) & 1);
      const int tiles = min(TPS, nt - st * TPS);
#pragma unroll
      for (int ti = 0; ti < TPS; ++ti) {
        if (ti < tiles) {
          const uint32_t wt = wring_u + slot * WSTAGE + ti * TILE_BYTES;
          if (A8) {
            const uint64_t bd = wg_desc(xring_u + xs * XSTAGE + (ti >> 1) * kTcXTile) + (uint64_t)(4 * (ti & 1));
            uint32_t a[2][4];
#pragma unroll
            for (int c = 0; c < 2; ++c) {
              const uint4 v0 = lds128(wt + off0[c]), v1 = lds128(wt + off1[c]);
              a[c][0] = nib4_to_e4m3(word(v0, wa), qsh, msel);
              a[c][1] = nib4_to_e4m3(word(v1, wa), qsh, msel);
              a[c][2] = nib4_to_e4m3(word(v0, 2 + wa), qsh, msel);
              a[c][3] = nib4_to_e4m3(word(v1, 2 + wa), qsh, msel);
            }
            wg_fence();
#pragma unroll
            for (int c = 0; c < 2; ++c) wg_mma<KIND>(dt, a[c], bd + (uint64_t)(2 * c), n32);
          } else {
            const uint64_t bd = wg_desc(xring_u + xs * XSTAGE + ti * kTcXTile);
            if (WBITS == 4) {
              uint32_t a[4][4];
#pragma unroll
              for (int c = 0; c < 2; ++c) {
                const uint4 v0 = lds128(wt + off0[c]), v1 = lds128(wt + off1[c]);
#pragma unroll
                for (int h = 0; h < 2; ++h) {
                  uint32_t* f = a[2 * c + h];
                  f[0] = lop3_and_or(__funnelshift_r(word(v0, 2 * h), word(v0, 2 * h), sh4), kMask4, F::kMagic);
                  f[1] = lop3_and_or(__funnelshift_r(word(v1, 2 * h), word(v1, 2 * h), sh4), kMask4, F::kMagic);
                  f[2] = lop3_and_or(__funnelshift_r(word(v0, 2 * h + 1), word(v0, 2 * h + 1), sh4), kMask4, F::kMagic);
                  f[3] = lop3_and_or(__funnelshift_r(word(v1, 2 * h + 1), word(v1, 2 * h + 1), sh4), kMask4, F::kMagic);
                  if (GROUPED) {
                    uint32_t sw[4], cw[4];
                    if (p.group_k > 0) {
#pragma unroll
                      for (int e = 0; e < 4; ++e) {
                        const int k0 = (kt0 + st * TPS + ti) * kBK + 32 * c + 8 * (2 * h + (e >> 1));
                        const float2 z = __ldg(p.sz + (size_t)min(k0 / p.group_k, p.ngroups - 1) * p.Np + ng * kBN + ((e & 1) ? rr1 : rr0));
                        sw[e] = F::pack(z.x, z.x);
                        const float cc = (F::kBias + 8.f - z.y) * z.x;
                        cw[e] = F::pack(cc, cc);
                      }
                    } else {
#pragma unroll
                      for (int e = 0; e < 4; ++e) {
                        if (DUAL) {
                          sw[e] = __byte_perm(gs2[ti][0], 0, (e & 1) ? 0x3232 : 0x1010);
                          cw[e] = __byte_perm(gc2[ti][0], 0, (e & 1) ? 0x3232 : 0x1010);
                        } else {
                          sw[e] = gs2[ti][e & 1]; cw[e] = gc2[ti][e & 1];
                        }
                      }
                    }
#pragma unroll
                    for (int e = 0; e < 4; ++e) {
                      uint32_t t2;
                      if (H) {
                        asm("add.rn.f16x2 %0, %1, %2;" : "=r"(t2) : "r"(f[e]), "r"(0xD840D840u));
                        asm("fma.rn.f16x2 %0, %1, %2, %3;" : "=r"(f[e]) : "r"(t2), "r"(sw[e]), "r"(cw[e]));
                      } else {
                        asm("add.rn.bf16x2 %0, %1, %2;" : "=r"(t2) : "r"(f[e]), "r"(0xC1C0C1C0u));
                        asm("fma.rn.bf16x2 %0, %1, %2, %3;" : "=r"(f[e]) : "r"(t2), "r"(sw[e]), "r"(cw[e]));
                      }
                    }
                  }
                }
                if (DUAL) {
                  wg_fence();
                  wg_mma<KIND>(d, a[2 * c], bd + (uint64_t)(4 * c), n32);
                  wg_mma<KIND>(d, a[2 * c + 1], bd + (uint64_t)(4 * c + 2), n32);
                  wg_commit();
                  wg_wait<1>();
                }
              }
              if (!DUAL) {
                wg_fence();
#pragma unroll
                for (int kk = 0; kk < 4; ++kk) wg_mma<KIND>(d, a[kk], bd + (uint64_t)(2 * kk), n32);
              }
            } else if (WBITS == 16) {
              uint32_t a[4][4];
#pragma unroll
              for (int kk = 0; kk < 4; ++kk) {
                a[kk][0] = lds32(wt + off0[2 * kk] + 4 * t4);
                a[kk][1] = lds32(wt + off1[2 * kk] + 4 * t4);
                a[kk][2] = lds32(wt + off0[2 * kk + 1] + 4 * t4);
                a[kk][3] = lds32(wt + off1[2 * kk + 1] + 4 * t4);
              }
              wg_fence();
#pragma unroll
              for (int kk = 0; kk < 4; ++kk) wg_mma<KIND>(d, a[kk], bd + (uint64_t)(2 * kk), n32);
            } else {
              uint32_t lo[4][4], hi[4][4];
#pragma unroll
              for (int c = 0; c < 4; ++c) {
                const uint4 v0 = lds128(wt + off0[c]), v1 = lds128(wt + off1[c]);
                const uint32_t w[4] = {word(v0, wa), word(v1, wa), word(v0, 2 + wa), word(v1, 2 + wa)};
#pragma unroll
                for (int e = 0; e < 4; ++e) {
                  lo[c][e] = lop3_and_or(__funnelshift_r(w[e], w[e], sh8), kMask4, F::kMagic);
                  hi[c][e] = lop3_and_or(__funnelshift_r(w[e], w[e], sh8 + 4), kMask4, F::kMagicHi);
                }
              }
              wg_fence();
#pragma unroll
              for (int c = 0; c < 4; ++c) {
                wg_mma<KIND>(d, lo[c], bd + (uint64_t)(2 * c), n32);
                wg_mma<KIND>(d, hi[c], bd + (uint64_t)(2 * c), n32);
              }
            }
          }
          if (!DUAL) {
            wg_commit();
            wg_wait<1>();
          }
          if (ti == 0 && prev_xs >= 0) {
            __syncwarp();
            if (lane == 0) mbar_arrive(&xfree[prev_xs]);
            prev_xs = -1;
          }
          if (A8 && ((ti & 1) || ti + 1 == tiles)) {
            wg_wait<0>();
            wg_fence_acc(dt);
#pragma unroll
            for (int i = 0; i < 32; ++i) { d[i] += dt[i]; dt[i] = 0.f; }
          }
        }
      }
      __syncwarp();
      if (lane == 0) mbar_arrive(&wfree[slot]);
      prev_xs = xs;
    }
    wg_wait<0>();
    wg_fence_acc(d);
    __syncwarp();
    if (prev_xs >= 0 && lane == 0) mbar_arrive(&xfree[prev_xs]);

    asm volatile("bar.sync 3, 320;" ::: "memory");
    float* fs = reinterpret_cast<float*>(xring);
#pragma unroll
    for (int j = 0; j < 8; ++j) {
      const int m = 8 * j + 2 * t4;
      float s0 = 1.f, s1 = 1.f;
      if (A8 || p.norm_sumsq) { s0 = ascale[m]; s1 = ascale[m + 1]; }
      const float zz0 = A8 ? sz0.y - 16.f : sz0.y, zz1 = A8 ? sz1.y - 16.f : sz1.y;
      const float sa0 = suma[m], sa1 = suma[m + 1];
      fs[m * kBN + rr0] = sz0.x * s0 * (d[4 * j + 0] - zz0 * sa0);
      fs[(m + 1) * kBN + rr0] = sz0.x * s1 * (d[4 * j + 1] - zz0 * sa1);
      fs[m * kBN + rr1] = sz1.x * s0 * (d[4 * j + 2] - zz1 * sa0);
      fs[(m + 1) * kBN + rr1] = sz1.x * s1 * (d[4 * j + 3] - zz1 * sa1);
    }
  }

  pdl_wait();
  __syncthreads();
  {
    constexpr int T = kTcThreads;
    const float4* fs4 = reinterpret_cast<const float4*>(xring);
    float4* fs4w = reinterpret_cast<float4*>(xring);
    const int units = p.M * (kBN / 4);
    constexpr int MPK4 = kTcNM * kBN / 4;
    bool finalize = true;
    if (p.S > 1) {
      float4* wsu = reinterpret_cast<float4*>(p.ws) + ((size_t)ng * p.S + s) * MPK4;
      for (int i = tid; i < units; i += T) wsu[i] = fs4[i];
      __threadfence();
      __syncthreads();
      if (tid == 0) {
        const unsigned prev = atomicAdd(&p.counters[ng], 1u);
        s_is_last = (prev == (unsigned)(p.S - 1));
      }
      __syncthreads();
      finalize = s_is_last != 0;
      if (finalize) {
        __threadfence();
        const float4* wsg = reinterpret_cast<const float4*>(p.ws) + (size_t)ng * p.S * MPK4;
        for (int i0 = tid; i0 < units; i0 += 2 * T) {
          float4 a[2];
          a[0] = a[1] = make_float4(0.f, 0.f, 0.f, 0.f);
          for (int s0 = 0; s0 < p.S; s0 += 8) {
            float4 b[2][8];
#pragma unroll
            for (int g = 0; g < 2; ++g)
#pragma unroll
              for (int u = 0; u < 8; ++u) {
                const int i = i0 + g * T;
                b[g][u] = (s0 + u < p.S && i < units) ? __ldcg(wsg + (size_t)(s0 + u) * MPK4 + i) : make_float4(0.f, 0.f, 0.f, 0.f);
              }
#pragma unroll
            for (int g = 0; g < 2; ++g)
#pragma unroll
              for (int u = 0; u < 8; ++u) { a[g].x += b[g][u].x; a[g].y += b[g][u].y; a[g].z += b[g][u].z; a[g].w += b[g][u].w; }
          }
#pragma unroll
          for (int g = 0; g < 2; ++g) {
            const int i = i0 + g * T;
            if (i < units) fs4w[i] = a[g];
          }
        }
        if (tid == 0) p.counters[ng] = 0;
        __syncthreads();
      }
    }
    if (finalize) {
      const bool vec_ok = (p.ldc & 3) == 0 && (reinterpret_cast<uintptr_t>(p.C) & 7) == 0;
      if (p.act == B2_ACT_SWIGLU) {
        const int su = p.M * 16;
#pragma unroll 1
        for (int i = tid; i < su; i += T) {
          const int m = i >> 4, nq = i & 15;
          const int nn = ng * 64 + nq * 4;
          if (nn >= p.N) continue;
          const float4 gv = fs4[m * 32 + nq], uv = fs4[m * 32 + 16 + nq];
          float v[4];
          v[0] = apply_act<B2_ACT_SILU>(gv.x * p.alpha) * (uv.x * p.alpha);
          v[1] = apply_act<B2_ACT_SILU>(gv.y * p.alpha) * (uv.y * p.alpha);
          v[2] = apply_act<B2_ACT_SILU>(gv.z * p.alpha) * (uv.z * p.alpha);
          v[3] = apply_act<B2_ACT_SILU>(gv.w * p.alpha) * (uv.w * p.alpha);
          __nv_bfloat16* cp = p.C + (int64_t)m * p.ldc + nn;
          if (vec_ok && nn + 3 < p.N) {
            *reinterpret_cast<uint2*>(cp) = make_uint2(F::pack(v[0], v[1]), F::pack(v[2], v[3]));
          } else {
#pragma unroll
            for (int e = 0; e < 4; ++e)
              if (nn + e < p.N) cp[e] = F::from_f(v[e]);
          }
        }
      } else if (p.act == B2_ACT_NONE && vec_ok && (p.N & 3) == 0 &&
                 (!p.residual || (reinterpret_cast<uintptr_t>(p.residual) & 7) == 0) &&
                 (!p.bias || (reinterpret_cast<uintptr_t>(p.bias) & 7) == 0)) {
        constexpr int UPT = (kTcNM * (kBN / 4) + T - 1) / T;
        uint2 res[UPT];
#pragma unroll
        for (int j = 0; j < UPT; ++j) {
          const int i = tid + j * T;
          const int m = i >> 5, nn = ng * kBN + (i & 31) * 4;
          res[j] = make_uint2(0u, 0u);
          if (p.residual && i < units && nn < p.N) res[j] = __ldg(reinterpret_cast<const uint2*>(p.residual + (int64_t)m * p.ldc + nn));
        }
#pragma unroll
        for (int j = 0; j < UPT; ++j) {
          const int i = tid + j * T;
          const int m = i >> 5, nn = ng * kBN + (i & 31) * 4;
          float ssq = 0.f;
          if (i < units && nn < p.N) {
            const float4 a = fs4[i];
            float v0 = a.x * p.alpha, v1 = a.y * p.alpha, v2 = a.z * p.alpha, v3 = a.w * p.alpha;
            if (p.bias) {
              const uint2 bv = __ldg(reinterpret_cast<const uint2*>(p.bias + nn));
              v0 += F::lo(bv.x); v1 += F::hi(bv.x); v2 += F::lo(bv.y); v3 += F::hi(bv.y);
            }
            v0 += F::lo(res[j].x); v1 += F::hi(res[j].x); v2 += F::lo(res[j].y); v3 += F::hi(res[j].y);
            const uint2 st2 = make_uint2(F::pack(v0, v1), F::pack(v2, v3));
            *reinterpret_cast<uint2*>(p.C + (int64_t)m * p.ldc + nn) = st2;
            if (p.xg_out) {
              const float r0 = F::lo(st2.x), r1 = F::hi(st2.x), r2 = F::lo(st2.y), r3 = F::hi(st2.y);
              const uint2 gv = __ldg(reinterpret_cast<const uint2*>(p.gamma_out + nn));
              *reinterpret_cast<uint2*>(p.xg_out + (int64_t)m * p.ldxg + nn) =
                  make_uint2(F::pack(r0 * F::lo(gv.x), r1 * F::hi(gv.x)), F::pack(r2 * F::lo(gv.y), r3 * F::hi(gv.y)));
              ssq = (r0 * r0 + r1 * r1) + (r2 * r2 + r3 * r3);
            }
          }
          if (p.xg_out) {
#pragma unroll
            for (int o = 16; o > 0; o >>= 1) ssq += __shfl_xor_sync(0xffffffffu, ssq, o);
            if (lane == 0 && i < units) p.sumsq_out[(size_t)ng * p.norm_ld + m] = ssq;
          }
        }
      } else {
        const float* fs = reinterpret_cast<const float*>(xring);
#pragma unroll 1
        for (int i = tid; i < p.M * (kBN / 2); i += T) {
          const int m = i >> 6, np = i & 63;
          const int nn = ng * kBN + np * 2;
          if (nn >= p.N) continue;
          float v0 = fs[m * kBN + np * 2] * p.alpha, v1 = fs[m * kBN + np * 2 + 1] * p.alpha;
          const bool has1 = (nn + 1) < p.N;
          if (p.bias) {
            v0 += F::to_f(p.bias[nn]);
            if (has1) v1 += F::to_f(p.bias[nn + 1]);
          }
          v0 = apply_act_rt(v0, p.act);
          v1 = apply_act_rt(v1, p.act);
          __nv_bfloat16* cp = p.C + (int64_t)m * p.ldc + nn;
          if (p.residual) {
            const __nv_bfloat16* rp = p.residual + (int64_t)m * p.ldc + nn;
            v0 += F::to_f(rp[0]);
            if (has1) v1 += F::to_f(rp[1]);
          }
          if (has1 && ((reinterpret_cast<uintptr_t>(cp) & 3) == 0)) {
            *reinterpret_cast<uint32_t*>(cp) = F::pack(v0, v1);
          } else {
            cp[0] = F::from_f(v0);
            if (has1) cp[1] = F::from_f(v1);
          }
        }
      }
    }
  }

  if (MULTI) asm volatile("fence.proxy.async.shared::cta;" ::: "memory");
  __syncthreads();
  }
}

int tc_smem_bytes(int wbits, bool dual) {
  const int tps = wbits == 4 ? (dual ? 2 : 4) : 2;
  const int wstage = tps * (wbits == 4 ? 4096 : (wbits == 8 ? 8192 : 16384));
  const int nsw = wbits == 16 ? 4 : kTcNSW;
  return 1024 + kTcNSX * tps * kTcXTile + nsw * wstage + kTcNM * 4 + 96 * 8 + 64;
}

EncodeTiledFn encode_tiled() {
  static EncodeTiledFn fn = nullptr;
  if (!fn) {
    void* p = nullptr;
    cudaDriverEntryPointQueryResult q;
    if (cudaGetDriverEntryPoint("cuTensorMapEncodeTiled", &p, cudaEnableDefault, &q) == cudaSuccess && q == cudaDriverEntryPointSuccess)
      fn = reinterpret_cast<EncodeTiledFn>(p);
  }
  return fn;
}

cudaError_t tc_launch(int wbits, const TcLaunch& a, cudaStream_t stream) {
  EncodeTiledFn enc = encode_tiled();
  if (!enc) return cudaErrorNotSupported;
  alignas(64) CUtensorMap amap;
  const bool a8 = a.a_scale != nullptr;
  const cuuint64_t gdim[2] = {(cuuint64_t)a.K, (cuuint64_t)a.M};
  const cuuint64_t gstride[1] = {(cuuint64_t)a.lda * (a8 ? 1 : 2)};
  static const int n32 = [] { const char* e = getenv("B2_GEMM_TC_N32"); return e ? atoi(e) : 1; }();
  const int nm = (n32 && a.M <= 32) ? 32 : kTcNM;
  const cuuint32_t box[2] = {(cuuint32_t)(a8 ? 2 * kBK : kBK), (cuuint32_t)nm};
  const cuuint32_t estr[2] = {1, 1};
  if (enc(&amap, a8 ? CU_TENSOR_MAP_DATA_TYPE_UINT8 : CU_TENSOR_MAP_DATA_TYPE_BFLOAT16, 2, const_cast<__nv_bfloat16*>(a.A), gdim, gstride, box, estr,
          CU_TENSOR_MAP_INTERLEAVE_NONE, CU_TENSOR_MAP_SWIZZLE_128B, CU_TENSOR_MAP_L2_PROMOTION_L2_128B,
          CU_TENSOR_MAP_FLOAT_OOB_FILL_NONE) != CUDA_SUCCESS)
    return cudaErrorInvalidValue;

  TcParams p;
  p.packed = a.packed; p.sz = a.sz; p.A = a.A; p.lda = a.lda; p.C = a.C; p.ldc = a.ldc; p.bias = a.bias; p.residual = a.residual;
  p.ws = a.ws; p.counters = a.counters; p.M = a.M; p.N = a.N; p.K = a.K; p.Np = a.Np; p.KT = a.KT; p.NG = a.NG; p.S = a.S;
  p.act = a.act; p.alpha = a.alpha;
  p.a_scale = a.a_scale; p.tile_sums = a.tile_sums;
  p.norm_sumsq = a.norm_sumsq; p.norm_parts = a.norm_parts; p.norm_ld = a.norm_ld; p.norm_inv_hidden = a.norm_inv_hidden;
  p.norm_eps = a.norm_eps; p.sumsq_out = a.sumsq_out; p.xg_out = a.xg_out; p.gamma_out = a.gamma_out; p.ldxg = a.ldxg;
  p.nm = nm; p.group_tiles = a.group_tiles; p.group_k = a.group_k; p.ngroups = a.ngroups;
  static const int persist = [] { const char* e = getenv("B2_GEMM_TC_PERSIST"); return e ? atoi(e) : 1; }();
  const int units = a.NG * a.S;
  const bool dual = a.dual && wbits == 4 && !a8;
  const int cap = (dual ? 2 : 1) * sm_count();
  const int grid = (persist && units > cap) ? cap : units;
  const bool multi = units > grid;
  const size_t smem = (size_t)tc_smem_bytes(wbits, dual);
  auto go = [&](auto kern) {
    const cudaError_t e = raise_smem_limit((const void*)kern, (int)smem);
    return e != cudaSuccess ? e : launch(kern, dim3(grid), dim3(kTcThreads), smem, stream, true, p, amap);
  };
  const bool g = a.group_tiles > 0 || a.group_k > 0, h = a.fp16;
  if (a8) {
    if (wbits != 4 || h) return cudaErrorNotSupported;
    return multi ? go(wq_gemm_tc_kernel<4, true, true>) : go(wq_gemm_tc_kernel<4, false, true>);
  }
  if (g && wbits != 4) return cudaErrorNotSupported;
  if (wbits == 4) {
    switch ((multi ? 8 : 0) | (g ? 4 : 0) | (dual ? 2 : 0) | (h ? 1 : 0)) {
      case 0: return go(wq_gemm_tc_kernel<4, false, false, false, false, false>);
      case 1: return go(wq_gemm_tc_kernel<4, false, false, false, false, true>);
      case 2: return go(wq_gemm_tc_kernel<4, false, false, false, true, false>);
      case 3: return go(wq_gemm_tc_kernel<4, false, false, false, true, true>);
      case 4: return go(wq_gemm_tc_kernel<4, false, false, true, false, false>);
      case 5: return go(wq_gemm_tc_kernel<4, false, false, true, false, true>);
      case 6: return go(wq_gemm_tc_kernel<4, false, false, true, true, false>);
      case 7: return go(wq_gemm_tc_kernel<4, false, false, true, true, true>);
      case 8: return go(wq_gemm_tc_kernel<4, true, false, false, false, false>);
      case 9: return go(wq_gemm_tc_kernel<4, true, false, false, false, true>);
      case 10: return go(wq_gemm_tc_kernel<4, true, false, false, true, false>);
      case 11: return go(wq_gemm_tc_kernel<4, true, false, false, true, true>);
      case 12: return go(wq_gemm_tc_kernel<4, true, false, true, false, false>);
      case 13: return go(wq_gemm_tc_kernel<4, true, false, true, false, true>);
      case 14: return go(wq_gemm_tc_kernel<4, true, false, true, true, false>);
      default: return go(wq_gemm_tc_kernel<4, true, false, true, true, true>);
    }
  }
  if (wbits == 16) {
    if (h) return multi ? go(wq_gemm_tc_kernel<16, true, false, false, false, true>) : go(wq_gemm_tc_kernel<16, false, false, false, false, true>);
    return multi ? go(wq_gemm_tc_kernel<16, true>) : go(wq_gemm_tc_kernel<16, false>);
  }
  if (h) return multi ? go(wq_gemm_tc_kernel<8, true, false, false, false, true>) : go(wq_gemm_tc_kernel<8, false, false, false, false, true>);
  return multi ? go(wq_gemm_tc_kernel<8, true>) : go(wq_gemm_tc_kernel<8, false>);
}

}
```

Baseline: 7110.

## Replace persistent/dual-CTA TC GEMM scheduling with stream-K tile partitioning and carry-over

Drops the dual-CTA-per-SM variant and the persistent multi-unit loop in the tensor-core weight-quantized GEMM. When N groups outnumber SMs, the total k-tile work is now divided evenly across CTAs stream-K style. A CTA whose range ends mid-group parks its partial accumulators and row sums in a per-CTA workspace slot and raises a flag. The next CTA spins on that flag, reloads the partials and finishes the group. The int4 weight ring is deepened to 10 stages with two tiles per stage, and the n32 choice becomes a compile-time template parameter. The aim is to remove wave-quantization imbalance across SMs, at the cost of a serialized spin-wait handoff between neighbouring CTAs and extra global traffic for the parked tiles.

```diff
diff --git a/dash-infer_b200/csrc/wq_gemm.cu b/dash-infer_b200/csrc/wq_gemm.cu
--- a/dash-infer_b200/csrc/wq_gemm.cu
+++ b/dash-infer_b200/csrc/wq_gemm.cu
@@ -791,8 +791,6 @@
   bool own_sz = false;
   unsigned* counters = nullptr;
   Plan plans[2];
-  int tc_S = 0;
-  int tc_S2 = 0;
   bool pair = false;
   int device = 0;
 };
@@ -1058,32 +1056,10 @@
   return M >= kTcMinM && (h->group_tiles == 0 || h->d.wbits == 4);
 }
 
-static int make_tc_plan(b2_gemm_wq* h) {
-  if (h->tc_S > 0) return B2_OK;
-  const int ctas = env_int("B2_GEMM_TC_CTAS_PER_SM", 1);
-  auto split_for = [&](int slots, int smax) {
-    int S = slots / h->NG;
-    if (S > h->KT / 4) S = h->KT / 4;
-    if (S > smax) S = smax;
-    return S < 1 ? 1 : S;
-  };
-  h->tc_S = split_for(ctas * sm_count(), env_int("B2_GEMM_TC_MAX_SPLIT", 6));
-  h->tc_S2 = split_for(env_int("B2_GEMM_TC_DUAL_SLOTS", 2) * sm_count(), env_int("B2_GEMM_TC_MAX_SPLIT2", 8));
-  return B2_OK;
-}
-
-static bool tc_dual(const b2_gemm_wq* h) {
-  static const int on = env_int("B2_GEMM_TC_DUAL", 1);
-  if (!on || h->d.wbits != 4) return false;
-  return on >= 2 || h->NG >= 2 * sm_count();
-}
-
 size_t b2_gemm_wq_workspace_bytes(b2_gemm_wq_t h, int M) {
   if (!h || M <= 0) return 0;
   if (use_tc(h, M)) {
-    if (make_tc_plan(h) != B2_OK) return 0;
-    const int sm = h->tc_S > h->tc_S2 ? h->tc_S : h->tc_S2;
-    return sm <= 1 ? 16 : (size_t)h->NG * sm * kTcMaxM * kBN * sizeof(float) + 16;
+    return tc_workspace_bytes(h->NG, h->KT);
   }
   const int mc = M > kGemvMaxM ? kGemvMaxM : M;
   const int mti = mt_index_for(mc);
@@ -1133,9 +1109,7 @@
   if (activation != B2_ACT_SWIGLU && (activation < 0 || activation > B2_ACT_SIGMOID)) return B2_ERR_PARAM;
   if (h->pair && (bias || residual)) return B2_ERR_UNSUPPORTED;
   if ((reinterpret_cast<uintptr_t>(A8) & 15) || (lda_bytes % 16) != 0 || lda_bytes < h->d.K) return B2_ERR_UNSUPPORTED;
-  if (int st = make_tc_plan(h)) return st;
-  const size_t need = h->tc_S <= 1 ? 16 : (size_t)h->NG * h->tc_S * kTcMaxM * kBN * sizeof(float) + 16;
-  if (workspace_bytes < need || (h->tc_S > 1 && !workspace)) return B2_ERR_PARAM;
+  if (workspace_bytes < tc_workspace_bytes(h->NG, h->KT) || !workspace) return B2_ERR_PARAM;
   for (int m0 = 0; m0 < M; m0 += kTcMaxM) {
     TcLaunch a;
     a.packed = (const uint8_t*)h->packed; a.sz = h->sz;
@@ -1145,7 +1119,7 @@
     a.residual = residual ? (const __nv_bfloat16*)residual + (int64_t)m0 * ldc : nullptr;
     a.ws = (float*)workspace; a.counters = h->counters;
     a.M = (M - m0) > kTcMaxM ? kTcMaxM : (M - m0);
-    a.N = h->d.N; a.K = h->d.K; a.Np = h->Np; a.KT = h->KT; a.NG = h->NG; a.S = h->tc_S;
+    a.N = h->d.N; a.K = h->d.K; a.Np = h->Np; a.KT = h->KT; a.NG = h->NG;
     a.act = activation; a.alpha = alpha;
     a.a_scale = a_scale + m0; a.tile_sums = tile_sums + (size_t)m0 * h->KT;
     cudaError_t e = tc_launch(4, a, (cudaStream_t)stream_);
@@ -1204,13 +1178,9 @@
   cudaStream_t stream = (cudaStream_t)stream_;
   const bool grouped = h->group_tiles > 0;
   if (use_tc(h, M) && !comm) {
-    if (int st = make_tc_plan(h)) return st;
-    const bool dual = tc_dual(h);
-    const int tcs = dual ? h->tc_S2 : h->tc_S;
-    if (tcs > 1 && !workspace) return B2_ERR_PARAM;
+    if (!workspace) return B2_ERR_PARAM;
     for (int m0 = 0; m0 < M; m0 += kTcMaxM) {
       TcLaunch a;
-      a.dual = dual;
       a.fp16 = h->d.ft == B2_DT_F16;
       a.packed = (const uint8_t*)h->packed; a.sz = h->sz;
       a.A = (const __nv_bfloat16*)A + (int64_t)m0 * lda; a.lda = lda;
@@ -1219,7 +1189,7 @@
       a.residual = residual ? (const __nv_bfloat16*)residual + (int64_t)m0 * ldc : nullptr;
       a.ws = (float*)workspace; a.counters = h->counters;
       a.M = (M - m0) > kTcMaxM ? kTcMaxM : (M - m0);
-      a.N = h->d.N; a.K = h->d.K; a.Np = h->Np; a.KT = h->KT; a.NG = h->NG; a.S = tcs;
+      a.N = h->d.N; a.K = h->d.K; a.Np = h->Np; a.KT = h->KT; a.NG = h->NG;
       a.act = activation; a.alpha = alpha;
       a.group_tiles = h->group_tiles;
       a.group_k = h->group_k; a.ngroups = h->G;
diff --git a/dash-infer_b200/csrc/wq_gemm_shared.cuh b/dash-infer_b200/csrc/wq_gemm_shared.cuh
--- a/dash-infer_b200/csrc/wq_gemm_shared.cuh
+++ b/dash-infer_b200/csrc/wq_gemm_shared.cuh
@@ -26,7 +26,7 @@
   const __nv_bfloat16* residual;
   float* ws;
   unsigned* counters;
-  int M, N, K, Np, KT, NG, S;
+  int M, N, K, Np, KT, NG;
   int act;
   float alpha;
   const float* a_scale = nullptr;
@@ -34,7 +34,6 @@
   int group_tiles = 0;
   int group_k = 0, ngroups = 1;
   bool fp16 = false;
-  bool dual = false;
   const float* norm_sumsq = nullptr;
   int norm_parts = 0, norm_ld = 0;
   float norm_inv_hidden = 0.f, norm_eps = 0.f;
@@ -64,7 +63,10 @@
 
 constexpr int kGemvMaxM = 16;
 constexpr int kTcMaxM = 64;
-int tc_smem_bytes(int wbits, bool dual);
+int tc_smem_bytes(int wbits);
+int tc_split(int NG, int KT);
+int tc_grid(int NG, int KT);
+size_t tc_workspace_bytes(int NG, int KT);
 cudaError_t tc_launch(int wbits, const TcLaunch& a, cudaStream_t stream);
 
 cudaError_t raise_smem_limit(const void* kern, int smem);
diff --git a/dash-infer_b200/csrc/wq_gemm_tc.cu b/dash-infer_b200/csrc/wq_gemm_tc.cu
--- a/dash-infer_b200/csrc/wq_gemm_tc.cu
+++ b/dash-infer_b200/csrc/wq_gemm_tc.cu
@@ -1,4 +1,5 @@
 #include <cstdlib>
+#include <type_traits>
 
 #include "b2_common.cuh"
 #include "wq_gemm_shared.cuh"
@@ -7,7 +8,8 @@
 
 constexpr int kTcThreads = 384;
 constexpr int kTcNM = 64;
-constexpr int kTcNSW = 6;
+constexpr int kTcNSW = 10;
+__host__ __device__ constexpr int tc_nsw(int wbits) { return wbits == 16 ? 4 : (wbits == 4 ? kTcNSW : 6); }
 constexpr int kTcNSX = 3;
 constexpr int kTcXTile = kTcNM * 128;
 
@@ -33,9 +35,9 @@
   B2_WG_ACC16(d), "+f"(d[16]), "+f"(d[17]), "+f"(d[18]), "+f"(d[19]), "+f"(d[20]), "+f"(d[21]), "+f"(d[22]), "+f"(d[23]), \
       "+f"(d[24]), "+f"(d[25]), "+f"(d[26]), "+f"(d[27]), "+f"(d[28]), "+f"(d[29]), "+f"(d[30]), "+f"(d[31])
 
-template <int KIND>
-__device__ __forceinline__ void wg_mma(float (&d)[32], const uint32_t (&a)[4], uint64_t desc, bool n32) {
-  if (n32) {
+template <int KIND, bool N32>
+__device__ __forceinline__ void wg_mma(float (&d)[32], const uint32_t (&a)[4], uint64_t desc) {
+  if (N32) {
     if (KIND == 0)
       asm volatile("{\n\t.reg .pred p;\n\tsetp.ne.b32 p, %21, 0;\n\t"
                    "wgmma.mma_async.sync.aligned.m64n32k16.f32.bf16.bf16 " B2_WG_D16 ", {%16,%17,%18,%19}, %20, p, 1, 1, 0;\n\t}"
@@ -83,6 +85,14 @@
   uint32_t r;
   asm("lop3.b32 %0, %1, %2, %3, 0xD8;" : "=r"(r) : "r"(lo), "r"(hi), "r"(m));
   return r;
+}
+
+constexpr int kTcContFloats = 256 * 32 + 4 * 64;
+
+__device__ __forceinline__ unsigned ld_acquire_u32(const unsigned* p) {
+  unsigned v;
+  asm volatile("ld.acquire.gpu.global.u32 %0, [%1];" : "=r"(v) : "l"(p) : "memory");
+  return v;
 }
 
 struct TcParams {
@@ -113,22 +123,21 @@
   int group_k, ngroups;
 };
 
-template <int WBITS, bool MULTI, bool A8 = false, bool GROUPED = false, bool DUAL = false, bool H = false>
-__global__ void __launch_bounds__(kTcThreads, DUAL ? 2 : 1) wq_gemm_tc_kernel(const TcParams p, const __grid_constant__ CUtensorMap amap) {
+template <int WBITS, bool A8 = false, bool GROUPED = false, bool H = false>
+__global__ void __launch_bounds__(kTcThreads, 1) wq_gemm_tc_kernel(const TcParams p, const __grid_constant__ CUtensorMap amap) {
   constexpr int TILE_BYTES = WBITS == 4 ? 4096 : (WBITS == 8 ? 8192 : 16384);
   constexpr int NCH = WBITS == 4 ? 2 : (WBITS == 8 ? 4 : 8);
-  constexpr int NSW = WBITS == 16 ? 4 : kTcNSW;
-  constexpr int TPS = WBITS == 4 ? (DUAL ? 2 : 4) : 2;
+  constexpr int NSW = tc_nsw(WBITS);
+  constexpr int TPS = 2;
   constexpr int KIND = A8 ? 2 : (H ? 1 : 0);
   static_assert(!A8 || WBITS == 4, "fp8 activations: int4 weights only");
-  static_assert(!DUAL || (WBITS == 4 && !A8), "two CTAs per SM: int4 weights, 16-bit activations");
   static_assert(!H || !A8, "fp8 activations come with bf16 outputs");
   using F = Ft<H>;
   static_assert(!GROUPED || (!A8 && WBITS != 16), "sub-channel weights: bf16 activations, int4 / int8");
   const int XTILE_LD = p.nm * 128;
-  constexpr int XTPS = A8 ? TPS / 2 : TPS;
   constexpr int WSTAGE = TPS * TILE_BYTES;
-  constexpr int XSTAGE = XTPS * kTcXTile;
+  constexpr int XSTAGE = TPS * kTcXTile;
+  static_assert(kTcNSX * XSTAGE >= kTcNM * kBN * 4, "the activation ring holds the parked fp32 tile");
   extern __shared__ uint8_t smem_raw[];
   uint8_t* smem = reinterpret_cast<uint8_t*>((reinterpret_cast<uintptr_t>(smem_raw) + 1023) & ~uintptr_t(1023));
   uint8_t* xring = smem;
@@ -144,7 +153,6 @@
   __shared__ int s_is_last;
 
   const int tid = threadIdx.x, warp = tid >> 5, lane = tid & 31;
-  const int nunits = p.NG * p.S;
 
   if (tid == 0) {
     for (int i = 0; i < NSW; ++i) { mbar_init(&wfull[i], 1); mbar_init(&wfree[i], 8); }
@@ -154,16 +162,54 @@
   __syncthreads();
   pdl_launch_dependents();
 
+  const int64_t W = (int64_t)p.NG * p.KT;
+  const int b = blockIdx.x, grid = gridDim.x;
+  int t_begin, t_end;
+  if (p.S > 1) {
+    const int ng = b / p.S, s = b - ng * p.S;
+    t_begin = ng * p.KT + (int)((int64_t)s * p.KT / p.S);
+    t_end = ng * p.KT + (int)((int64_t)(s + 1) * p.KT / p.S);
+  } else if (A8) {
+    t_begin = p.KT * (int)((int64_t)p.NG * b / grid);
+    t_end = p.KT * (int)((int64_t)p.NG * (b + 1) / grid);
+  } else {
+    t_begin = (int)(W * b / grid);
+    t_end = (int)(W * (b + 1) / grid);
+  }
+  const bool tail_first = p.S == 1 && t_begin % p.KT != 0;
+  const int t_main = tail_first ? (t_begin / p.KT + 1) * p.KT : t_begin;
+  const int n_main = t_main < t_end ? (t_end - 1) / p.KT - t_main / p.KT + 1 : 0;
+  const int npieces = n_main + (tail_first ? 1 : 0);
+  auto piece_at = [&](int i, int& pa, int& pe) {
+    if (i < n_main) {
+      pa = i == 0 ? t_main : (t_main / p.KT + i) * p.KT;
+      pe = min(t_end, (t_main / p.KT + i + 1) * p.KT);
+    } else {
+      pa = t_begin;
+      pe = t_main;
+    }
+  };
+  float* cont = p.ws + (size_t)b * kTcContFloats;
+  int gbase = 0;
   int w_pre = 0;
-  const int my_units = !MULTI ? 1 : ((int)blockIdx.x < nunits) ? (nunits - (int)blockIdx.x + (int)gridDim.x - 1) / (int)gridDim.x : 0;
-  for (int uit = 0; uit < my_units; ++uit) {
-  const int unit = (int)blockIdx.x + uit * (int)gridDim.x;
-  const int ng = unit / p.S;
-  const int s = unit - ng * p.S;
-  const int kt0 = (int)((int64_t)s * p.KT / p.S), kt1 = (int)((int64_t)(s + 1) * p.KT / p.S);
+  for (int pi = 0; pi < npieces; ++pi) {
+  int ta, te;
+  piece_at(pi, ta, te);
+  const int ng = ta / p.KT;
+  const int kt0 = ta - ng * p.KT, kt1 = te - ng * p.KT;
   const int nt = kt1 - kt0;
   const int nst = (nt + TPS - 1) / TPS;
-  const int gbase = MULTI ? uit * nst : 0;
+  const bool head = p.S == 1 && kt1 != p.KT;
+  const bool tail = p.S == 1 && kt0 != 0;
+  if (tail && (warp < 8 || warp >= 10)) {
+    if (tid == 0) {
+      pdl_wait();
+      while (ld_acquire_u32(&p.counters[ng]) == 0) __nanosleep(64);
+      p.counters[ng] = 0;
+    }
+    asm volatile("bar.sync 3, 320;" ::: "memory");
+  }
+  const float* cont_in = cont - kTcContFloats;
   if (warp == 8) {
     if (lane == 0) {
       auto issue = [&](int g, const uint8_t* src, uint32_t bytes) {
@@ -172,18 +218,16 @@
         mbar_arrive_expect_tx(&wfull[slot], bytes);
         bulk_g2s(wring + slot * WSTAGE, src, bytes, &wfull[slot]);
       };
-      const uint8_t* wsrc = p.packed + ((size_t)ng * p.KT + kt0) * TILE_BYTES;
+      const uint8_t* wsrc = p.packed + (size_t)ta * TILE_BYTES;
       for (int st = w_pre; st < nst; ++st) issue(gbase + st, wsrc + (size_t)st * WSTAGE, min(TPS, nt - st * TPS) * TILE_BYTES);
       w_pre = 0;
-      const int nu = unit + gridDim.x;
-      if (MULTI && nu < nunits) {
-        const int ng2 = nu / p.S, s2 = nu - ng2 * p.S;
-        const int k0 = (int)((int64_t)s2 * p.KT / p.S), k1 = (int)((int64_t)(s2 + 1) * p.KT / p.S);
-        const int nt2 = k1 - k0, nst2 = (nt2 + TPS - 1) / TPS;
-        const uint8_t* wsrc2 = p.packed + ((size_t)ng2 * p.KT + k0) * TILE_BYTES;
+      if (pi + 1 < npieces) {
+        int ta2, te2;
+        piece_at(pi + 1, ta2, te2);
+        const int nt2 = te2 - ta2, nst2 = (nt2 + TPS - 1) / TPS;
         w_pre = min(NSW, nst2);
         for (int st = 0; st < w_pre; ++st)
-          issue(gbase + nst + st, wsrc2 + (size_t)st * WSTAGE, min(TPS, nt2 - st * TPS) * TILE_BYTES);
+          issue(gbase + nst + st, p.packed + (size_t)ta2 * TILE_BYTES + (size_t)st * WSTAGE, min(TPS, nt2 - st * TPS) * TILE_BYTES);
       }
     }
   } else if (warp == 9) {
@@ -210,6 +254,10 @@
   } else if (warp >= 10) {
     const int xt = tid - 320;
     float r0 = 0.f, r1 = 0.f, r2 = 0.f, r3 = 0.f;
+    if (tail) {
+      r0 = __ldcg(cont_in + 8192 + xt); r1 = __ldcg(cont_in + 8192 + 64 + xt);
+      r2 = __ldcg(cont_in + 8192 + 128 + xt); r3 = __ldcg(cont_in + 8192 + 192 + xt);
+    }
     if (A8) {
       pdl_wait();
       if (xt < p.M) {
@@ -247,12 +295,15 @@
       __syncwarp();
       if (lane == 0) mbar_arrive(&xsum[slot]);
     }
+    if (head) {
+      pdl_wait();
+      cont[8192 + xt] = r0; cont[8192 + 64 + xt] = r1; cont[8192 + 128 + xt] = r2; cont[8192 + 192 + xt] = r3;
+    }
     suma[xt] = (r0 + r1) + (r2 + r3);
     asm volatile("bar.sync 3, 320;" ::: "memory");
   } else {
     const int wg = warp >> 2, g8 = lane >> 2, t4 = lane & 3;
     const int rr0 = wg * 64 + (warp & 3) * 16 + g8, rr1 = rr0 + 8;
-    const bool n32 = p.nm == 32;
     const float2 sz0 = (WBITS == 16 || GROUPED) ? make_float2(1.f, 0.f) : p.sz[ng * kBN + rr0];
     const float2 sz1 = (WBITS == 16 || GROUPED) ? make_float2(1.f, 0.f) : p.sz[ng * kBN + rr1];
     const uint32_t wring_u = smem_u32(wring), xring_u = smem_u32(xring);
@@ -268,8 +319,15 @@
 
     float d[32], dt[32];
 #pragma unroll
-    for (int i = 0; i < 32; ++i) d[i] = dt[i] = 0.f;
+    for (int i = 0; i < 32; ++i) {
+      d[i] = tail ? __ldcg(cont_in + i * 256 + tid) : 0.f;
+      dt[i] = 0.f;
+    }
     int prev_xs = -1;
+    auto main_loop = [&](auto n32c) {
+    constexpr bool N32 = decltype(n32c)::value;
+    uint32_t fa[2][4][4];
+    uint32_t flo[2][4][4], fhi[2][4][4];
     for (int st = 0; st < nst; ++st) {
       const int g = gbase + st;
       const int slot = g % NSW, xs = g % kTcNSX;
@@ -281,13 +339,8 @@
           const float2 z0 = __ldg(p.sz + (size_t)(kt / p.group_tiles) * p.Np + ng * kBN + rr0);
           const float2 z1 = __ldg(p.sz + (size_t)(kt / p.group_tiles) * p.Np + ng * kBN + rr1);
           const float c0 = (F::kBias + 8.f - z0.y) * z0.x, c1 = (F::kBias + 8.f - z1.y) * z1.x;
-          if (DUAL) {
-            gs2[ti][0] = F::pack(z0.x, z1.x);
-            gc2[ti][0] = F::pack(c0, c1);
-          } else {
-            gs2[ti][0] = F::pack(z0.x, z0.x); gs2[ti][1] = F::pack(z1.x, z1.x);
-            gc2[ti][0] = F::pack(c0, c0); gc2[ti][1] = F::pack(c1, c1);
-          }
+          gs2[ti][0] = F::pack(z0.x, z0.x); gs2[ti][1] = F::pack(z1.x, z1.x);
+          gc2[ti][0] = F::pack(c0, c0); gc2[ti][1] = F::pack(c1, c1);
         }
       }
       mbar_wait(&wfull[slot], (g / NSW) & 1);
@@ -299,7 +352,7 @@
           const uint32_t wt = wring_u + slot * WSTAGE + ti * TILE_BYTES;
           if (A8) {
             const uint64_t bd = wg_desc(xring_u + xs * XSTAGE + (ti >> 1) * kTcXTile) + (uint64_t)(4 * (ti & 1));
-            uint32_t a[2][4];
+            uint32_t (&a)[4][4] = fa[ti & 1];
 #pragma unroll
             for (int c = 0; c < 2; ++c) {
               const uint4 v0 = lds128(wt + off0[c]), v1 = lds128(wt + off1[c]);
@@ -310,11 +363,11 @@
             }
             wg_fence();
 #pragma unroll
-            for (int c = 0; c < 2; ++c) wg_mma<KIND>(dt, a[c], bd + (uint64_t)(2 * c), n32);
+            for (int c = 0; c < 2; ++c) wg_mma<KIND, N32>(dt, a[c], bd + (uint64_t)(2 * c));
           } else {
             const uint64_t bd = wg_desc(xring_u + xs * XSTAGE + ti * kTcXTile);
             if (WBITS == 4) {
-              uint32_t a[4][4];
+              uint32_t (&a)[4][4] = fa[ti & 1];
 #pragma unroll
               for (int c = 0; c < 2; ++c) {
                 const uint4 v0 = lds128(wt + off0[c]), v1 = lds128(wt + off1[c]);
@@ -338,14 +391,7 @@
                       }
                     } else {
 #pragma unroll
-                      for (int e = 0; e < 4; ++e) {
-                        if (DUAL) {
-                          sw[e] = __byte_perm(gs2[ti][0], 0, (e & 1) ? 0x3232 : 0x1010);
-                          cw[e] = __byte_perm(gc2[ti][0], 0, (e & 1) ? 0x3232 : 0x1010);
-                        } else {
-                          sw[e] = gs2[ti][e & 1]; cw[e] = gc2[ti][e & 1];
-                        }
-                      }
+                      for (int e = 0; e < 4; ++e) { sw[e] = gs2[ti][e & 1]; cw[e] = gc2[ti][e & 1]; }
                     }
 #pragma unroll
                     for (int e = 0; e < 4; ++e) {
@@ -360,21 +406,12 @@
                     }
                   }
                 }
-                if (DUAL) {
-                  wg_fence();
-                  wg_mma<KIND>(d, a[2 * c], bd + (uint64_t)(4 * c), n32);
-                  wg_mma<KIND>(d, a[2 * c + 1], bd + (uint64_t)(4 * c + 2), n32);
-                  wg_commit();
-                  wg_wait<1>();
-                }
               }
-              if (!DUAL) {
-                wg_fence();
-#pragma unroll
-                for (int kk = 0; kk < 4; ++kk) wg_mma<KIND>(d, a[kk], bd + (uint64_t)(2 * kk), n32);
-              }
+              wg_fence();
+#pragma unroll
+              for (int kk = 0; kk < 4; ++kk) wg_mma<KIND, N32>(d, a[kk], bd + (uint64_t)(2 * kk));
             } else if (WBITS == 16) {
-              uint32_t a[4][4];
+              uint32_t (&a)[4][4] = fa[ti & 1];
 #pragma unroll
               for (int kk = 0; kk < 4; ++kk) {
                 a[kk][0] = lds32(wt + off0[2 * kk] + 4 * t4);
@@ -384,9 +421,10 @@
               }
               wg_fence();
 #pragma unroll
-              for (int kk = 0; kk < 4; ++kk) wg_mma<KIND>(d, a[kk], bd + (uint64_t)(2 * kk), n32);
+              for (int kk = 0; kk < 4; ++kk) wg_mma<KIND, N32>(d, a[kk], bd + (uint64_t)(2 * kk));
             } else {
-              uint32_t lo[4][4], hi[4][4];
+              uint32_t (&lo)[4][4] = flo[ti & 1];
+              uint32_t (&hi)[4][4] = fhi[ti & 1];
 #pragma unroll
               for (int c = 0; c < 4; ++c) {
                 const uint4 v0 = lds128(wt + off0[c]), v1 = lds128(wt + off1[c]);
@@ -400,15 +438,13 @@
               wg_fence();
 #pragma unroll
               for (int c = 0; c < 4; ++c) {
-                wg_mma<KIND>(d, lo[c], bd + (uint64_t)(2 * c), n32);
-                wg_mma<KIND>(d, hi[c], bd + (uint64_t)(2 * c), n32);
+                wg_mma<KIND, N32>(d, lo[c], bd + (uint64_t)(2 * c));
+                wg_mma<KIND, N32>(d, hi[c], bd + (uint64_t)(2 * c));
               }
             }
           }
-          if (!DUAL) {
-            wg_commit();
-            wg_wait<1>();
-          }
+          wg_commit();
+          wg_wait<1>();
           if (ti == 0 && prev_xs >= 0) {
             __syncwarp();
             if (lane == 0) mbar_arrive(&xfree[prev_xs]);
@@ -428,13 +464,21 @@
     }
     wg_wait<0>();
     wg_fence_acc(d);
+    };
+    if (p.nm == 32) main_loop(std::true_type());
+    else main_loop(std::false_type());
     __syncwarp();
     if (prev_xs >= 0 && lane == 0) mbar_arrive(&xfree[prev_xs]);
 
     asm volatile("bar.sync 3, 320;" ::: "memory");
+    if (head) {
+      pdl_wait();
+#pragma unroll
+      for (int i = 0; i < 32; ++i) cont[i * 256 + tid] = d[i];
+    }
     float* fs = reinterpret_cast<float*>(xring);
 #pragma unroll
-    for (int j = 0; j < 8; ++j) {
+    for (int j = 0; j < 8 && !head; ++j) {
       const int m = 8 * j + 2 * t4;
       float s0 = 1.f, s1 = 1.f;
       if (A8 || p.norm_sumsq) { s0 = ascale[m]; s1 = ascale[m + 1]; }
@@ -455,15 +499,20 @@
     float4* fs4w = reinterpret_cast<float4*>(xring);
     const int units = p.M * (kBN / 4);
     constexpr int MPK4 = kTcNM * kBN / 4;
-    bool finalize = true;
-    if (p.S > 1) {
-      float4* wsu = reinterpret_cast<float4*>(p.ws) + ((size_t)ng * p.S + s) * MPK4;
+    bool finalize = !head;
+    if (head) {
+      __threadfence();
+      __syncthreads();
+      if (tid == 0) atomicExch(&p.counters[ng], 1u);
+    } else if (p.S > 1) {
+      const int np = p.S;
+      float4* wsu = reinterpret_cast<float4*>(p.ws) + (size_t)b * MPK4;
       for (int i = tid; i < units; i += T) wsu[i] = fs4[i];
       __threadfence();
       __syncthreads();
       if (tid == 0) {
         const unsigned prev = atomicAdd(&p.counters[ng], 1u);
-        s_is_last = (prev == (unsigned)(p.S - 1));
+        s_is_last = (prev == (unsigned)(np - 1));
       }
       __syncthreads();
       finalize = s_is_last != 0;
@@ -473,14 +522,14 @@
         for (int i0 = tid; i0 < units; i0 += 2 * T) {
           float4 a[2];
           a[0] = a[1] = make_float4(0.f, 0.f, 0.f, 0.f);
-          for (int s0 = 0; s0 < p.S; s0 += 8) {
+          for (int s0 = 0; s0 < np; s0 += 8) {
             float4 b[2][8];
 #pragma unroll
             for (int g = 0; g < 2; ++g)
 #pragma unroll
               for (int u = 0; u < 8; ++u) {
                 const int i = i0 + g * T;
-                b[g][u] = (s0 + u < p.S && i < units) ? __ldcg(wsg + (size_t)(s0 + u) * MPK4 + i) : make_float4(0.f, 0.f, 0.f, 0.f);
+                b[g][u] = (s0 + u < np && i < units) ? __ldcg(wsg + (size_t)(s0 + u) * MPK4 + i) : make_float4(0.f, 0.f, 0.f, 0.f);
               }
 #pragma unroll
             for (int g = 0; g < 2; ++g)
@@ -594,16 +643,15 @@
     }
   }
 
-  if (MULTI) asm volatile("fence.proxy.async.shared::cta;" ::: "memory");
+  asm volatile("fence.proxy.async.shared::cta;" ::: "memory");
   __syncthreads();
-  }
-}
-
-int tc_smem_bytes(int wbits, bool dual) {
-  const int tps = wbits == 4 ? (dual ? 2 : 4) : 2;
-  const int wstage = tps * (wbits == 4 ? 4096 : (wbits == 8 ? 8192 : 16384));
-  const int nsw = wbits == 16 ? 4 : kTcNSW;
-  return 1024 + kTcNSX * tps * kTcXTile + nsw * wstage + kTcNM * 4 + 96 * 8 + 64;
+  gbase += nst;
+  }
+}
+
+int tc_smem_bytes(int wbits) {
+  const int wstage = 2 * (wbits == 4 ? 4096 : (wbits == 8 ? 8192 : 16384));
+  return 1024 + kTcNSX * 2 * kTcXTile + tc_nsw(wbits) * wstage + kTcNM * 4 + 96 * 8 + 64;
 }
 
 EncodeTiledFn encode_tiled() {
@@ -635,19 +683,14 @@
 
   TcParams p;
   p.packed = a.packed; p.sz = a.sz; p.A = a.A; p.lda = a.lda; p.C = a.C; p.ldc = a.ldc; p.bias = a.bias; p.residual = a.residual;
-  p.ws = a.ws; p.counters = a.counters; p.M = a.M; p.N = a.N; p.K = a.K; p.Np = a.Np; p.KT = a.KT; p.NG = a.NG; p.S = a.S;
+  p.ws = a.ws; p.counters = a.counters; p.M = a.M; p.N = a.N; p.K = a.K; p.Np = a.Np; p.KT = a.KT; p.NG = a.NG; p.S = tc_split(a.NG, a.KT);
   p.act = a.act; p.alpha = a.alpha;
   p.a_scale = a.a_scale; p.tile_sums = a.tile_sums;
   p.norm_sumsq = a.norm_sumsq; p.norm_parts = a.norm_parts; p.norm_ld = a.norm_ld; p.norm_inv_hidden = a.norm_inv_hidden;
   p.norm_eps = a.norm_eps; p.sumsq_out = a.sumsq_out; p.xg_out = a.xg_out; p.gamma_out = a.gamma_out; p.ldxg = a.ldxg;
   p.nm = nm; p.group_tiles = a.group_tiles; p.group_k = a.group_k; p.ngroups = a.ngroups;
-  static const int persist = [] { const char* e = getenv("B2_GEMM_TC_PERSIST"); return e ? atoi(e) : 1; }();
-  const int units = a.NG * a.S;
-  const bool dual = a.dual && wbits == 4 && !a8;
-  const int cap = (dual ? 2 : 1) * sm_count();
-  const int grid = (persist && units > cap) ? cap : units;
-  const bool multi = units > grid;
-  const size_t smem = (size_t)tc_smem_bytes(wbits, dual);
+  const int grid = tc_grid(a.NG, a.KT);
+  const size_t smem = (size_t)tc_smem_bytes(wbits);
   auto go = [&](auto kern) {
     const cudaError_t e = raise_smem_limit((const void*)kern, (int)smem);
     return e != cudaSuccess ? e : launch(kern, dim3(grid), dim3(kTcThreads), smem, stream, true, p, amap);
@@ -655,35 +698,33 @@
   const bool g = a.group_tiles > 0 || a.group_k > 0, h = a.fp16;
   if (a8) {
     if (wbits != 4 || h) return cudaErrorNotSupported;
-    return multi ? go(wq_gemm_tc_kernel<4, true, true>) : go(wq_gemm_tc_kernel<4, false, true>);
+    return go(wq_gemm_tc_kernel<4, true>);
   }
   if (g && wbits != 4) return cudaErrorNotSupported;
   if (wbits == 4) {
-    switch ((multi ? 8 : 0) | (g ? 4 : 0) | (dual ? 2 : 0) | (h ? 1 : 0)) {
-      case 0: return go(wq_gemm_tc_kernel<4, false, false, false, false, false>);
-      case 1: return go(wq_gemm_tc_kernel<4, false, false, false, false, true>);
-      case 2: return go(wq_gemm_tc_kernel<4, false, false, false, true, false>);
-      case 3: return go(wq_gemm_tc_kernel<4, false, false, false, true, true>);
-      case 4: return go(wq_gemm_tc_kernel<4, false, false, true, false, false>);
-      case 5: return go(wq_gemm_tc_kernel<4, false, false, true, false, true>);
-      case 6: return go(wq_gemm_tc_kernel<4, false, false, true, true, false>);
-      case 7: return go(wq_gemm_tc_kernel<4, false, false, true, true, true>);
-      case 8: return go(wq_gemm_tc_kernel<4, true, false, false, false, false>);
-      case 9: return go(wq_gemm_tc_kernel<4, true, false, false, false, true>);
-      case 10: return go(wq_gemm_tc_kernel<4, true, false, false, true, false>);
-      case 11: return go(wq_gemm_tc_kernel<4, true, false, false, true, true>);
-      case 12: return go(wq_gemm_tc_kernel<4, true, false, true, false, false>);
-      case 13: return go(wq_gemm_tc_kernel<4, true, false, true, false, true>);
-      case 14: return go(wq_gemm_tc_kernel<4, true, false, true, true, false>);
-      default: return go(wq_gemm_tc_kernel<4, true, false, true, true, true>);
-    }
-  }
-  if (wbits == 16) {
-    if (h) return multi ? go(wq_gemm_tc_kernel<16, true, false, false, false, true>) : go(wq_gemm_tc_kernel<16, false, false, false, false, true>);
-    return multi ? go(wq_gemm_tc_kernel<16, true>) : go(wq_gemm_tc_kernel<16, false>);
-  }
-  if (h) return multi ? go(wq_gemm_tc_kernel<8, true, false, false, false, true>) : go(wq_gemm_tc_kernel<8, false, false, false, false, true>);
-  return multi ? go(wq_gemm_tc_kernel<8, true>) : go(wq_gemm_tc_kernel<8, false>);
-}
-
-}
+    if (g) return h ? go(wq_gemm_tc_kernel<4, false, true, true>) : go(wq_gemm_tc_kernel<4, false, true>);
+    return h ? go(wq_gemm_tc_kernel<4, false, false, true>) : go(wq_gemm_tc_kernel<4>);
+  }
+  if (wbits == 16) return h ? go(wq_gemm_tc_kernel<16, false, false, true>) : go(wq_gemm_tc_kernel<16>);
+  return h ? go(wq_gemm_tc_kernel<8, false, false, true>) : go(wq_gemm_tc_kernel<8>);
+}
+
+int tc_split(int NG, int KT) {
+  int S = sm_count() / NG;
+  if (S > KT / 4) S = KT / 4;
+  if (S > 6) S = 6;
+  return S < 1 ? 1 : S;
+}
+
+int tc_grid(int NG, int KT) {
+  const int S = tc_split(NG, KT);
+  return S > 1 ? NG * S : (NG < sm_count() ? NG : sm_count());
+}
+
+size_t tc_workspace_bytes(int NG, int KT) {
+  const int S = tc_split(NG, KT);
+  if (S > 1) return (size_t)NG * S * kTcMaxM * kBN * sizeof(float) + 16;
+  return (size_t)tc_grid(NG, KT) * kTcContFloats * sizeof(float) + 16;
+}
+
+}
```

After: 7425 (median of 6 runs). 1.04x the previous value.
